# Liaoyongjian1/HC-MVS

Measured on AMD Instinct MI355X. Metric: PatchMatch Mpix/s (1080p, 8 views, 7x7, 8 iter), higher is better.
Workload: dtype f32; 1 GPU; batch of 32 independent units per GPU, each 1 ref x 8 src views, 1920x1080, 7x7 taps (adapthalfwin 6), 8 sweeps, it_external 0, full EstimateDepthMap (median + init score + sweeps + end pass); batch=32, exchange=none

## Files before the change

hc-mvs_amd/csrc/hcmvs_api.cpp:

```cpp
#include "../../include/hcmvs_hip.h"
#include "pm_common.h"
#include "fuse_common.h"
#include "pf_chain.h"
#include "filter_plan.h"
#include "tri_init.h"
#include "cloud_kernels.h"
#include "vis_kernels.h"
#include "dev_buf.h"

#include <cmath>
#include <cstdarg>
#include <cstdio>
#include <cstring>
#include <map>
#include <string>
#include <algorithm>
#include <chrono>
#include <vector>

using namespace hcmvs;

namespace {

constexpr int kMaxBatch = HCMVS_MAX_BATCH;

struct View {
	View() = default;
	explicit View(Reclaimer* r) : grayMem(r), bgrMem(r), gra(r), keep(r), quads(r), depthMem(r), normalMem(r), confMem(r), dNeighbors(r) {}
	int w = 0, h = 0;
	float* gray = nullptr;
	uint8_t* bgr = nullptr;
	DevBuf grayMem, bgrMem;
	DevBuf gra;
	DevBuf keep;
	DevBuf quads;
	double K[9], R[9], C[3];
	float *mDepth = nullptr, *mNormal = nullptr, *mConf = nullptr;
	DevBuf depthMem, normalMem, confMem;
	float dMin = 0.f, dMax = 0.f;
	DevBuf dNeighbors;
	std::vector<uint32_t> neighbors;
	const float *sDepth = nullptr, *sNormal = nullptr, *sConf = nullptr;
	bool rescaled = false;
};

}


struct hcmvs_ctx final : Reclaimer {
	int device = 0;
	hipStream_t ownStream = nullptr;
	hipStream_t stream = nullptr;
	std::string err;
	std::map<uint32_t, View> views;
	struct Slot {
		explicit Slot(Reclaimer* r) : dn(r), conf(r), tmpDepth(r), progress(r), srcSlab(r) {}
		DevBuf dn, conf, tmpDepth;
		DevBuf progress;
		DevBuf srcSlab;
	};
	std::vector<Slot> slots;
	DevBuf tmpU8{this};
	DevBuf maskStage{this};
	DevBuf sDepth{this}, sNormal{this}, sConf{this};
	DevBuf dViews{this};
	std::vector<DevView> hViews;
	DevBuf dItems{this};
	std::vector<EstConst> hItems;
	DevBuf dSpread{this};
	std::vector<SpreadView> hSpread;
	int viewspread = 0;
	bool haveSpreadStats = false;
	DevBuf sync{this};
	int sweepPerLaunch = 0;
	DevBuf evals{this};
	hipEvent_t ev[4] = {nullptr, nullptr, nullptr, nullptr};
	int lastSweeps = 0, lastSweepLaunches = 0;
	bool haveStats = false;
	int sweepLag = 1;
	int sweepSegment = -1;
	int fuseOrder = 0;
	int xcdAffinity = 1;
	DevBuf dMaps{this};
	DevBuf counters{this};
	DevBuf fuseScratch{this};
	DevBuf filterStage{this}, filterTab{this}, filterCnt{this};
	DevBuf passScratch{this};
	DevBuf pfState;
	bool errPending = false;
	int nCU = 0;
	hipEvent_t upEv[2] = {nullptr, nullptr};
	char* pinned = nullptr; size_t capPinned = 0;
	int wavesPerRow = 0;

	bool reclaim() override {
		if (!pfState.capacity()) return false;
		(void)hipStreamSynchronize(stream);
		pfState.reset();
		return true;
	}
};

static int fail(hcmvs_ctx* c, int code, const char* fmt, ...) {
	if (c) {
		char buf[512];
		va_list ap;
		va_start(ap, fmt);
		vsnprintf(buf, sizeof buf, fmt, ap);
		va_end(ap);
		c->err = buf;
	}
	return code;
}
#define HIPCHK(c, call)                                                                             \
	do {                                                                                            \
		hipError_t e_ = (call);                                                                     \
		if (e_ != hipSuccess) return fail(c, HCMVS_ERR_HIP, "%s: %s", #call, hipGetErrorString(e_)); \
	} while (0)

static void mat3_mul(const double* a, const double* b, double* c) {
	for (int i = 0; i < 3; ++i)
		for (int j = 0; j < 3; ++j) {
			double s = 0;
			for (int k = 0; k < 3; ++k) s += a[i * 3 + k] * b[k * 3 + j];
			c[i * 3 + j] = s;
		}
}
static void mat3_mul_bt(const double* a, const double* b, double* c) {
	for (int i = 0; i < 3; ++i)
		for (int j = 0; j < 3; ++j) {
			double s = 0;
			for (int k = 0; k < 3; ++k) s += a[i * 3 + k] * b[j * 3 + k];
			c[i * 3 + j] = s;
		}
}
static void mat3_inv(const double* m, double* r) {
	const double d = m[0] * (m[4] * m[8] - m[5] * m[7]) - m[1] * (m[3] * m[8] - m[5] * m[6]) +
	                 m[2] * (m[3] * m[7] - m[4] * m[6]);
	const double id = 1.0 / d;
	r[0] = (m[4] * m[8] - m[5] * m[7]) * id;
	r[1] = (m[2] * m[7] - m[1] * m[8]) * id;
	r[2] = (m[1] * m[5] - m[2] * m[4]) * id;
	r[3] = (m[5] * m[6] - m[3] * m[8]) * id;
	r[4] = (m[0] * m[8] - m[2] * m[6]) * id;
	r[5] = (m[2] * m[3] - m[0] * m[5]) * id;
	r[6] = (m[3] * m[7] - m[4] * m[6]) * id;
	r[7] = (m[1] * m[6] - m[0] * m[7]) * id;
	r[8] = (m[0] * m[4] - m[1] * m[3]) * id;
}
static inline float fd2r(float d) { return d * (3.14159274101257324f / 180.f); }

#ifdef HCMVS_STAMPS
namespace hcmvs { void debug_read_stamps(unsigned long long* out, int reset); }
#endif
namespace hcmvs {
void launch_resize_gray(const float* src, int sw, int sh, float* dst, int dw, int dh, float scaleParam, hipStream_t s);
void launch_ignore_mask(const uint16_t* labels, int lw, int lh, const int32_t* ignore, int nIgnore, uint8_t* keep, int W, int H, hipStream_t s);
}

extern "C" {

void hcmvs_default_params(hcmvs_params* p) {
	if (!p) return;
	memset(p, 0, sizeof *p);
	p->adapthalfwin = 5;
	p->n_estimation_iters = 1;
	p->it_external = 0;
	p->n_external_iters = 1;
	p->propagate_halfwin = 1;
	p->propagate_step = 4;
	p->n_random_iters = 6;
	p->ncc_threshold_keep = 0.55f;
	p->random_depth_ratio = 0.003f;
	p->random_angle1_deg = 16.f;
	p->random_angle2_deg = 10.f;
	p->random_smooth_depth = 0.02f;
	p->random_smooth_normal_deg = 13.f;
	p->random_smooth_bonus = 0.93f;
	p->photometric_flow = 0.f;
	p->seed = 1234;
	p->median_blur = 1;
}

int hcmvs_create(int device, hcmvs_ctx** out) {
	if (!out) return HCMVS_ERR_INVALID;
	*out = nullptr;
	int n = 0;
	if (hipGetDeviceCount(&n) != hipSuccess || n <= 0 || device < 0 || device >= n) return HCMVS_ERR_NO_DEVICE;
	if (hipSetDevice(device) != hipSuccess) return HCMVS_ERR_NO_DEVICE;
	hipDeviceProp_t prop;
	if (hipGetDeviceProperties(&prop, device) != hipSuccess) return HCMVS_ERR_NO_DEVICE;
	if (strncmp(prop.gcnArchName, "gfx950", 6) != 0) return HCMVS_ERR_NO_DEVICE;
	hcmvs_ctx* c = new hcmvs_ctx();
	c->device = device;
	c->nCU = prop.multiProcessorCount;
	if (hipStreamCreateWithFlags(&c->ownStream, hipStreamNonBlocking) != hipSuccess) { hcmvs_destroy(c); return HCMVS_ERR_NO_DEVICE; }
	c->stream = c->ownStream;
	for (auto& e : c->ev)
		if (hipEventCreate(&e) != hipSuccess) { hcmvs_destroy(c); return HCMVS_ERR_NO_DEVICE; }
	c->hViews.resize((size_t)kMaxBatch * kMaxViews); c->hItems.resize(kMaxBatch); c->hSpread.resize((size_t)kMaxBatch * kMaxViews);
	if (c->dViews.reserve(sizeof(DevView) * kMaxViews * kMaxBatch, c->stream) != hipSuccess || c->evals.reserve(64, c->stream) != hipSuccess ||
	    c->dSpread.reserve(sizeof(SpreadView) * kMaxViews * kMaxBatch, c->stream) != hipSuccess ||
	    c->dItems.reserve(sizeof(EstConst) * kMaxBatch, c->stream) != hipSuccess || c->sync.reserve(64 + sizeof(int32_t) * 2 * kMaxBatch, c->stream) != hipSuccess) {
		hcmvs_destroy(c);
		return HCMVS_ERR_NO_DEVICE;
	}
	const char* lag = getenv("HCMVS_SWEEP_LAG");
	if (lag && atoi(lag) >= 1) c->sweepLag = atoi(lag);
	const char* aff = getenv("HCMVS_XCD_AFFINITY");
	if (aff) c->xcdAffinity = atoi(aff) != 0;
	const char* spl = getenv("HCMVS_SWEEP_LAUNCHES");
	if (spl && strcmp(spl, "per-sweep") == 0) c->sweepPerLaunch = 1;
	if (spl && strcmp(spl, "one") == 0) c->sweepPerLaunch = 2;
	const char* sgl = getenv("HCMVS_SWEEP_SEGMENT");
	if (sgl && atoi(sgl) >= 0) c->sweepSegment = atoi(sgl);
	const char* wpr = getenv("HCMVS_WAVES_PER_ROW");
	if (wpr && (atoi(wpr) == 1 || atoi(wpr) == 2 || atoi(wpr) == 3 || atoi(wpr) == 4)) c->wavesPerRow = atoi(wpr);
	*out = c;
	return HCMVS_OK;
}

void hcmvs_destroy(hcmvs_ctx* c) {
	if (!c) return;
	(void)hipSetDevice(c->device);
	(void)hipStreamSynchronize(c->stream);
	for (auto& e : c->ev) if (e) (void)hipEventDestroy(e);
	if (c->pinned) (void)hipHostFree(c->pinned);
	for (auto& e : c->upEv) if (e) (void)hipEventDestroy(e);
	if (c->ownStream) (void)hipStreamDestroy(c->ownStream);
	delete c;
}

const char* hcmvs_last_error(const hcmvs_ctx* c) { return c ? c->err.c_str() : "null context"; }

static int check_sweep_error(hcmvs_ctx* c) {
	if (!c->errPending) return HCMVS_OK;
	int32_t flags[2] = {0, 0};
	HIPCHK(c, hipMemcpy(flags, c->sync.get(), sizeof flags, hipMemcpyDeviceToHost));
	c->errPending = false;
	if (flags[1] != 0) return fail(c, HCMVS_ERR_TIMEOUT, "sweep worker timed out waiting for its predecessor row; the maps of the last estimate are incomplete");
	return HCMVS_OK;
}

int hcmvs_set_stream(hcmvs_ctx* c, void* stream) {
	if (!c) return HCMVS_ERR_INVALID;
	c->stream = stream ? (hipStream_t)stream : c->ownStream;
	return HCMVS_OK;
}
int hcmvs_synchronize(hcmvs_ctx* c) {
	if (!c) return HCMVS_ERR_INVALID;
	HIPCHK(c, hipSetDevice(c->device));
	HIPCHK(c, hipStreamSynchronize(c->stream));
	return check_sweep_error(c);
}

static int upload_staged(hcmvs_ctx* c, void* dst, const void* src, size_t bytes) {
	{
		hipPointerAttribute_t at;
		if (hipPointerGetAttributes(&at, src) == hipSuccess && at.type == hipMemoryTypeHost) {
			HIPCHK(c, hipMemcpyAsync(dst, src, bytes, hipMemcpyHostToDevice, c->stream));
			HIPCHK(c, hipStreamSynchronize(c->stream));
			return HCMVS_OK;
		}
		(void)hipGetLastError();
	}
	const size_t piece = (size_t)32 << 20;
	if (c->capPinned < 2 * piece) {
		if (c->pinned) (void)hipHostFree(c->pinned);
		c->pinned = nullptr; c->capPinned = 0;
		if (hipHostMalloc((void**)&c->pinned, 2 * piece, hipHostMallocDefault) != hipSuccess) {
			(void)hipGetLastError();
			HIPCHK(c, hipMemcpyAsync(dst, src, bytes, hipMemcpyHostToDevice, c->stream));
			HIPCHK(c, hipStreamSynchronize(c->stream));
			return HCMVS_OK;
		}
		c->capPinned = 2 * piece;
	}
	for (auto& e : c->upEv) if (!e) HIPCHK(c, hipEventCreateWithFlags(&e, hipEventDisableTiming));
	hipEvent_t done[2] = {c->upEv[0], c->upEv[1]};
	bool used[2] = {false, false};
	int k = 0;
	for (size_t off = 0; off < bytes; off += piece, k ^= 1) {
		const size_t n = std::min(piece, bytes - off);
		if (used[k]) HIPCHK(c, hipEventSynchronize(done[k]));
		memcpy(c->pinned + (size_t)k * piece, (const char*)src + off, n);
		HIPCHK(c, hipMemcpyAsync((char*)dst + off, c->pinned + (size_t)k * piece, n, hipMemcpyHostToDevice, c->stream));
		HIPCHK(c, hipEventRecord(done[k], c->stream));
		used[k] = true;
	}
	HIPCHK(c, hipStreamSynchronize(c->stream));
	return HCMVS_OK;
}

static int set_view(hcmvs_ctx* c, uint32_t id, int w, int h, const float* gray, const uint8_t* bgr, const double* K,
                    const double* R, const double* C, bool copy) {
	if (!c) return HCMVS_ERR_INVALID;
	if ((!gray && !bgr) || !K || !R || !C || w < 2 * kHalfWindow + 2 || h < 2 * kHalfWindow + 2 || w > 32768 || h > 32768 || id >= 65536)
		return fail(c, HCMVS_ERR_INVALID, "upload_view: bad arguments (id %u, %dx%d)", id, w, h);
	HIPCHK(c, hipSetDevice(c->device));
	auto it = c->views.find(id);
	if (it != c->views.end()) { HIPCHK(c, hipStreamSynchronize(c->stream)); it->second = View(c); }
	View v(c);
	v.w = w; v.h = h;
	const size_t n = (size_t)w * h;
	if (copy) {
		if (gray) {
			HIPCHK(c, v.grayMem.reserve(n * sizeof(float), c->stream));
			v.gray = v.grayMem.get<float>();
			const int rc = upload_staged(c, v.gray, gray, n * sizeof(float));
			if (rc) return rc;
		}
		if (bgr) {
			HIPCHK(c, v.bgrMem.reserve(n * 3, c->stream));
			v.bgr = v.bgrMem.get<uint8_t>();
			const int rc = upload_staged(c, v.bgr, bgr, n * 3);
			if (rc) return rc;
		}
	} else {
		v.gray = const_cast<float*>(gray);
		v.bgr = const_cast<uint8_t*>(bgr);
	}
	memcpy(v.K, K, sizeof v.K); memcpy(v.R, R, sizeof v.R); memcpy(v.C, C, sizeof v.C);
	c->views[id] = std::move(v);
	return HCMVS_OK;
}

int hcmvs_upload_view(hcmvs_ctx* c, uint32_t id, int32_t w, int32_t h, const float* gray, const uint8_t* bgr,
                      const double K[9], const double R[9], const double C[3]) {
	return set_view(c, id, w, h, gray, bgr, K, R, C, true);
}
int hcmvs_set_view_device(hcmvs_ctx* c, uint32_t id, int32_t w, int32_t h, const float* gray, const uint8_t* bgr,
                          const double K[9], const double R[9], const double C[3]) {
	return set_view(c, id, w, h, gray, bgr, K, R, C, false);
}
int hcmvs_rescale_view(hcmvs_ctx* c, uint32_t src_id, uint32_t dst_id, float scale) {
	if (!c) return HCMVS_ERR_INVALID;
	auto it = c->views.find(src_id);
	if (it == c->views.end() || dst_id >= 65536 || dst_id == src_id) return fail(c, HCMVS_ERR_INVALID, "rescale_view: bad view ids %u -> %u", src_id, dst_id);
	if (!(scale > 0.f) || fabsf(scale - 1.f) < 0.15f) return fail(c, HCMVS_ERR_INVALID, "rescale_view: scale %g is within 15 %% of 1 (DepthMap.h:234: not resampled)", scale);
	const View& src = it->second;
	if (!src.gray) return fail(c, HCMVS_ERR_INVALID, "rescale_view: view %u has no gray image (fuse-only view)", src_id);
	const int nw = (int)lrint((double)src.w * (double)scale), nh = (int)lrint((double)src.h * (double)scale);
	if (nw < 2 * kHalfWindow + 2 || nh < 2 * kHalfWindow + 2 || nw > 32768 || nh > 32768) return fail(c, HCMVS_ERR_INVALID, "rescale_view: %dx%d x %g gives an unusable size", src.w, src.h, scale);
	HIPCHK(c, hipSetDevice(c->device));
	auto old = c->views.find(dst_id);
	if (old != c->views.end()) { HIPCHK(c, hipStreamSynchronize(c->stream)); c->views.erase(old); }
	View v(c);
	v.w = nw; v.h = nh;
	HIPCHK(c, v.grayMem.reserve((size_t)nw * nh * sizeof(float), c->stream));
	v.gray = v.grayMem.get<float>();
	hcmvs::launch_resize_gray(src.gray, src.w, src.h, v.gray, nw, nh, scale, c->stream);
	HIPCHK(c, hipGetLastError());
	const double f = (double)std::max(nw, nh) / (double)std::max(src.w, src.h);
	memcpy(v.K, src.K, sizeof v.K); memcpy(v.R, src.R, sizeof v.R); memcpy(v.C, src.C, sizeof v.C);
	v.K[0] *= f; v.K[4] *= f; v.K[2] *= f; v.K[5] *= f;
	v.rescaled = true;
	c->views[dst_id] = std::move(v);
	return HCMVS_OK;
}
int hcmvs_get_view_info(hcmvs_ctx* c, uint32_t id, int32_t* w, int32_t* h, double K[9]) {
	if (!c) return HCMVS_ERR_INVALID;
	auto it = c->views.find(id);
	if (it == c->views.end()) return fail(c, HCMVS_ERR_INVALID, "get_view_info: unknown view %u", id);
	if (w) *w = it->second.w;
	if (h) *h = it->second.h;
	if (K) memcpy(K, it->second.K, sizeof(double) * 9);
	return HCMVS_OK;
}
int hcmvs_get_view_gray(hcmvs_ctx* c, uint32_t id, float* out) {
	if (!c || !out) return HCMVS_ERR_INVALID;
	auto it = c->views.find(id);
	if (it == c->views.end() || !it->second.gray) return fail(c, HCMVS_ERR_INVALID, "get_view_gray: unknown view %u (or a fuse-only view)", id);
	HIPCHK(c, hipSetDevice(c->device));
	HIPCHK(c, hipMemcpyAsync(out, it->second.gray, (size_t)it->second.w * it->second.h * sizeof(float), hipMemcpyDeviceToHost, c->stream));
	HIPCHK(c, hipStreamSynchronize(c->stream));
	return HCMVS_OK;
}

int hcmvs_release_view(hcmvs_ctx* c, uint32_t id) {
	if (!c) return HCMVS_ERR_INVALID;
	auto it = c->views.find(id);
	if (it == c->views.end()) return fail(c, HCMVS_ERR_INVALID, "release_view: unknown view %u", id);
	HIPCHK(c, hipSetDevice(c->device));
	HIPCHK(c, hipStreamSynchronize(c->stream));
	c->views.erase(it);
	return HCMVS_OK;
}

static int ensure_slot(hcmvs_ctx* c, int i, size_t n, int rows) {
	while ((int)c->slots.size() <= i) c->slots.emplace_back(c);
	hcmvs_ctx::Slot& sl = c->slots[i];
	HIPCHK(c, sl.dn.reserve(n * sizeof(float4), c->stream));
	HIPCHK(c, sl.conf.reserve(n * sizeof(float), c->stream));
	HIPCHK(c, sl.tmpDepth.reserve(n * sizeof(float), c->stream));
	HIPCHK(c, sl.progress.reserve((size_t)rows * kProgressStride * sizeof(int32_t), c->stream));
	return HCMVS_OK;
}

static int ensure_gradient(hcmvs_ctx* c, View& v) {
	if (v.gra.capacity()) return HCMVS_OK;
	const int n = v.w * v.h;
	HIPCHK(c, c->tmpU8.reserve((size_t)n, c->stream));
	HIPCHK(c, v.gra.reserve((size_t)n, c->stream));
	if (v.bgr) launch_bgr_to_u8(v.bgr, c->tmpU8.get<uint8_t>(), n, c->stream);
	else launch_gray_to_u8(v.gray, c->tmpU8.get<uint8_t>(), n, c->stream);
	launch_gradient_map(c->tmpU8.get<uint8_t>(), v.gra.get<uint8_t>(), v.w, v.h, c->stream);
	HIPCHK(c, hipGetLastError());
	return HCMVS_OK;
}

static int ensure_quads(hcmvs_ctx* c, View& v) {
	if (v.quads.capacity()) return HCMVS_OK;
	HIPCHK(c, v.quads.reserve((size_t)v.w * v.h * sizeof(float4), c->stream));
	launch_quads(v.gray, v.quads.get<float4>(), v.w, v.h, c->stream);
	HIPCHK(c, hipGetLastError());
	return HCMVS_OK;
}

int hcmvs_get_gradient_map(hcmvs_ctx* c, uint32_t id, uint8_t* out) {
	if (!c || !out) return HCMVS_ERR_INVALID;
	auto it = c->views.find(id);
	if (it == c->views.end()) return fail(c, HCMVS_ERR_INVALID, "get_gradient_map: unknown view %u", id);
	HIPCHK(c, hipSetDevice(c->device));
	int rc = ensure_gradient(c, it->second);
	if (rc) return rc;
	HIPCHK(c, hipMemcpyAsync(out, it->second.gra.get(), (size_t)it->second.w * it->second.h, hipMemcpyDeviceToHost, c->stream));
	HIPCHK(c, hipStreamSynchronize(c->stream));
	return HCMVS_OK;
}

static int set_ignore_mask(hcmvs_ctx* c, uint32_t id, const uint16_t* labels, int32_t lw, int32_t lh, const int32_t* ignore, int32_t nIgnore,
                           bool device) {
	if (!c) return HCMVS_ERR_INVALID;
	auto it = c->views.find(id);
	if (it == c->views.end()) return fail(c, HCMVS_ERR_INVALID, "set_ignore_mask: unknown view %u", id);
	View& v = it->second;
	HIPCHK(c, hipSetDevice(c->device));
	if (!labels) {
		HIPCHK(c, hipStreamSynchronize(c->stream));
		v.keep.reset();
		return HCMVS_OK;
	}
	if (lw < 1 || lh < 1 || lw > 65536 || lh > 65536 || nIgnore < 0 || (nIgnore > 0 && !ignore))
		return fail(c, HCMVS_ERR_INVALID, "set_ignore_mask: bad arguments (view %u, label image %dx%d, %d labels)", id, lw, lh, nIgnore);
	std::vector<int32_t> lab;
	for (int i = 0; i < nIgnore; ++i)
		if (ignore[i] >= 0 && ignore[i] <= 65535 && std::find(lab.begin(), lab.end(), ignore[i]) == lab.end()) lab.push_back(ignore[i]);
	const size_t imgBytes = (size_t)lw * lh * sizeof(uint16_t);
	Carve cv;
	const size_t oImg = device ? 0 : cv(imgBytes), oLab = cv(sizeof(int32_t) * (lab.size() + 1));
	HIPCHK(c, c->maskStage.reserve(cv.size, c->stream));
	HIPCHK(c, v.keep.reserve((size_t)v.w * v.h, c->stream));
	const uint16_t* dLabels = labels;
	if (!device) {
		const int rc = upload_staged(c, c->maskStage.get() + oImg, labels, imgBytes);
		if (rc) return rc;
		dLabels = (const uint16_t*)(c->maskStage.get() + oImg);
	}
	int32_t* dIgnore = (int32_t*)(c->maskStage.get() + oLab);
	if (!lab.empty()) HIPCHK(c, hipMemcpyAsync(dIgnore, lab.data(), sizeof(int32_t) * lab.size(), hipMemcpyHostToDevice, c->stream));
	launch_ignore_mask(dLabels, lw, lh, dIgnore, (int)lab.size(), v.keep.get<uint8_t>(), v.w, v.h, c->stream);
	HIPCHK(c, hipGetLastError());
	HIPCHK(c, hipStreamSynchronize(c->stream));
	return HCMVS_OK;
}

int hcmvs_set_ignore_mask(hcmvs_ctx* c, uint32_t id, const uint16_t* labels, int32_t lw, int32_t lh, const int32_t* ignore, int32_t n_ignore) {
	return set_ignore_mask(c, id, labels, lw, lh, ignore, n_ignore, false);
}
int hcmvs_set_ignore_mask_device(hcmvs_ctx* c, uint32_t id, const uint16_t* d_labels, int32_t lw, int32_t lh, const int32_t* ignore,
                                 int32_t n_ignore) {
	return set_ignore_mask(c, id, d_labels, lw, lh, ignore, n_ignore, true);
}
int hcmvs_get_ignore_mask(hcmvs_ctx* c, uint32_t id, uint8_t* keep) {
	if (!c || !keep) return HCMVS_ERR_INVALID;
	auto it = c->views.find(id);
	if (it == c->views.end()) return fail(c, HCMVS_ERR_INVALID, "get_ignore_mask: unknown view %u", id);
	const View& v = it->second;
	if (!v.keep.capacity()) { memset(keep, 1, (size_t)v.w * v.h); return HCMVS_OK; }
	HIPCHK(c, hipSetDevice(c->device));
	HIPCHK(c, hipMemcpyAsync(keep, v.keep.get(), (size_t)v.w * v.h, hipMemcpyDeviceToHost, c->stream));
	HIPCHK(c, hipStreamSynchronize(c->stream));
	return HCMVS_OK;
}

static int build_item(hcmvs_ctx* c, int slot, const hcmvs_batch_item& it, const hcmvs_params* p, EstConst& k) {
	if (!it.src_ids || !it.d_depth || !it.d_normal || !it.d_conf) return fail(c, HCMVS_ERR_INVALID, "estimate: null argument");
	const int n_src = it.n_src;
	if (n_src < 1 || n_src > HCMVS_MAX_VIEWS) return fail(c, HCMVS_ERR_INVALID, "estimate: n_src %d not in 1..%d", n_src, HCMVS_MAX_VIEWS);
	if (!(it.d_min >= 0.f) || !(it.d_max > it.d_min)) return fail(c, HCMVS_ERR_INVALID, "estimate: bad depth range [%g,%g)", it.d_min, it.d_max);
	auto rit = c->views.find(it.ref_id);
	if (rit == c->views.end()) return fail(c, HCMVS_ERR_INVALID, "estimate: unknown reference view %u", it.ref_id);
	View& ref = rit->second;
	if (!ref.gray) return fail(c, HCMVS_ERR_INVALID, "estimate: view %u was registered without a gray image (fuse-only view)", it.ref_id);
	int rc = ensure_slot(c, slot, (size_t)ref.w * ref.h, ref.h);
	if (rc) return rc;
	rc = ensure_gradient(c, ref);
	if (rc) return rc;
	memset(&k, 0, sizeof k);
	k.W = ref.w; k.H = ref.h; k.V = n_src;
	k.border = p->adapthalfwin > kHalfWindow ? p->adapthalfwin : kHalfWindow;
	if (ref.w < 2 * k.border + 2 || ref.h < 2 * k.border + 2) return fail(c, HCMVS_ERR_INVALID, "estimate: view %u (%dx%d) has no pixel inside the %d px border", it.ref_id, ref.w, ref.h, k.border);
	k.adapthalfwin = p->adapthalfwin; k.nRandomIters = p->n_random_iters; k.itExternal = p->it_external;
	k.propHalfwin = p->propagate_halfwin; k.propStep = p->propagate_step;
	k.ref = ref.gray; k.gra = ref.gra.get<uint8_t>(); k.views = c->dViews.get<DevView>() + (size_t)slot * kMaxViews;
	double Hr[9];
	mat3_inv(ref.K, Hr);
	for (int i = 0; i < 9; ++i) k.Hr[i] = (float)Hr[i];
	k.ifx = 1.0 / ref.K[0]; k.ify = 1.0 / ref.K[4]; k.cx = ref.K[2]; k.cy = ref.K[5];
	DevView* hv = c->hViews.data() + (size_t)slot * kMaxViews;
	memset(hv, 0, sizeof(DevView) * kMaxViews);
	uintptr_t lo = ~(uintptr_t)0, hi = 0;
	for (int v = 0; v < n_src; ++v) {
		auto sit = c->views.find(it.src_ids[v]);
		if (sit == c->views.end()) return fail(c, HCMVS_ERR_INVALID, "estimate: unknown source view %u", it.src_ids[v]);
		View& s = sit->second;
		if (!s.gray) return fail(c, HCMVS_ERR_INVALID, "estimate: source view %u was registered without a gray image (fuse-only view)", it.src_ids[v]);
		rc = ensure_quads(c, s);
		if (rc) return rc;
		double KR[9], Hl[9], A[9];
		mat3_mul(s.K, s.R, KR);
		mat3_mul_bt(KR, ref.R, Hl);
		const double dC[3] = {ref.C[0] - s.C[0], ref.C[1] - s.C[1], ref.C[2] - s.C[2]};
		for (int i = 0; i < 3; ++i) hv[v].Hm[i] = (float)(KR[i * 3] * dC[0] + KR[i * 3 + 1] * dC[1] + KR[i * 3 + 2] * dC[2]);
		mat3_mul(Hl, Hr, A);
		for (int i = 0; i < 9; ++i) hv[v].A[i] = (float)A[i];
		hv[v].w = s.w; hv[v].h = s.h;
		const uintptr_t b = (uintptr_t)s.quads.get(), e = b + (size_t)s.w * s.h * sizeof(float4);
		if (b < lo) lo = b;
		if (e > hi) hi = e;
	}
	if (hi - lo < 0xFFFF0000ull) {
		k.imgBase = (const char*)lo;
		for (int v = 0; v < n_src; ++v) hv[v].byteOff = (uint32_t)((uintptr_t)c->views.find(it.src_ids[v])->second.quads.get() - lo);
	} else {
		Carve slab;
		for (int v = 0; v < n_src; ++v) { const View& s = c->views.find(it.src_ids[v])->second; hv[v].byteOff = (uint32_t)slab((size_t)s.w * s.h * sizeof(float4)); }
		if (slab.size >= 0xFFFF0000ull) return fail(c, HCMVS_ERR_INVALID, "estimate: the source images of one item exceed 4 GiB");
		DevBuf& srcSlab = c->slots[slot].srcSlab;
		HIPCHK(c, srcSlab.reserve(slab.size, c->stream));
		for (int v = 0; v < n_src; ++v) {
			const View& s = c->views.find(it.src_ids[v])->second;
			HIPCHK(c, hipMemcpyAsync(srcSlab.get() + hv[v].byteOff, s.quads.get(), (size_t)s.w * s.h * sizeof(float4), hipMemcpyDeviceToDevice, c->stream));
		}
		k.imgBase = srcSlab.get();
	}
	k.dMin = it.d_min; k.dMax = it.d_max; k.dMinSqr = sqrtf(it.d_min); k.dMaxSqr = sqrtf(it.d_max);
	k.smoothBonusDepth = 1.f - p->random_smooth_bonus;
	k.smoothBonusNormal = (1.f - p->random_smooth_bonus) * 0.96f;
	k.smoothSigmaDepth = -1.f / (2.f * (p->random_smooth_depth * p->random_smooth_depth));
	{ const float r = fd2r(p->random_smooth_normal_deg); k.smoothSigmaNormal = -1.f / (2.f * (r * r)); }
	k.angle1Range = fd2r(p->random_angle1_deg);
	k.angle2Range = fd2r(p->random_angle2_deg);
	k.thConfSmall = p->ncc_threshold_keep * 0.2f;
	k.thConfBig = p->ncc_threshold_keep * 0.4f;
	k.thConfRand = p->ncc_threshold_keep * 0.9f;
	k.thRobust = p->ncc_threshold_keep * 1.2f;
	k.thKeep = p->ncc_threshold_keep;
	k.depthRatio = p->random_depth_ratio;
	k.pfScale = 1.f - p->photometric_flow;
	k.seed = p->seed + it.seed_offset;
	k.dn = c->slots[slot].dn.get<float4>(); k.conf = c->slots[slot].conf.get<float>(); k.progress = c->slots[slot].progress.get<int32_t>();
	k.hintDepth = nullptr; k.hintNormal = nullptr; k.hintIter = -1;
	if (it.d_hint_depth && it.d_hint_normal && p->it_external == p->n_external_iters - 1) {
		k.hintDepth = it.d_hint_depth; k.hintNormal = it.d_hint_normal; k.hintIter = p->n_estimation_iters - 1;
	}
	k.keep = ref.keep.capacity() ? ref.keep.get<uint8_t>() : nullptr;
	k.spread = nullptr;
	SpreadView* hs = c->hSpread.data() + (size_t)slot * kMaxViews;
	memset(hs, 0, sizeof(SpreadView) * kMaxViews);
	if (c->viewspread && p->it_external >= 1) {
		bool any = false;
		for (int v = 0; v < n_src; ++v) {
			const View& s = c->views.find(it.src_ids[v])->second;
			if (!s.sDepth || s.rescaled) continue;
			any = true;
			hs[v].depth = s.sDepth; hs[v].normal = s.sNormal; hs[v].conf = s.sConf;
			hs[v].w = s.w; hs[v].h = s.h;
			hs[v].cx = s.K[2]; hs[v].cy = s.K[5]; hs[v].ifx = 1.0 / s.K[0]; hs[v].ify = 1.0 / s.K[4];
			double T[9];
			mat3_mul_bt(ref.R, s.R, T);
			const double dC[3] = {s.C[0] - ref.C[0], s.C[1] - ref.C[1], s.C[2] - ref.C[2]};
			hs[v].Tz[0] = T[6]; hs[v].Tz[1] = T[7]; hs[v].Tz[2] = T[8];
			hs[v].tz = ref.R[6] * dC[0] + ref.R[7] * dC[1] + ref.R[8] * dC[2];
		}
		if (any) k.spread = c->dSpread.get<SpreadView>() + (size_t)slot * kMaxViews;
	}
	return HCMVS_OK;
}

static inline bool overlaps(const void* a, size_t na, const void* b, size_t nb) {
	const uintptr_t a0 = (uintptr_t)a, b0 = (uintptr_t)b;
	return a0 < b0 + nb && b0 < a0 + na;
}

static int check_spread_overlap(hcmvs_ctx* c, const hcmvs_batch_item* items, int n_items) {
	for (int i = 0; i < n_items; ++i) {
		const size_t n = (size_t)c->hItems[i].W * c->hItems[i].H;
		for (int k = 0; k < n_items; ++k)
			for (int v = 0; v < items[k].n_src; ++v) {
				const SpreadView& sv = c->hSpread[(size_t)k * kMaxViews + v];
				if (!c->hItems[k].spread || !sv.depth) continue;
				const size_t m = (size_t)sv.w * sv.h;
				const void* io[3] = {items[i].d_depth, items[i].d_normal, items[i].d_conf};
				const size_t ion[3] = {n * 4, n * 12, n * 4};
				const void* sp[3] = {sv.depth, sv.normal, sv.conf};
				const size_t spn[3] = {m * 4, m * 12, m * 4};
				for (int a = 0; a < 3; ++a)
					for (int b = 0; b < 3; ++b)
						if (overlaps(io[a], ion[a], sp[b], spn[b]))
							return fail(c, HCMVS_ERR_INVALID, "estimate: the in/out maps of item %d (view %u) overlap the spread maps of source view %u of item %d: "
							            "a launch must not read what it writes (register a copy, or estimate the two images in separate calls)", i, items[i].ref_id, items[k].src_ids[v], k);
			}
	}
	return HCMVS_OK;
}

int hcmvs_estimate_batch_device(hcmvs_ctx* c, const hcmvs_batch_item* items, int32_t n_items, const hcmvs_params* p) {
	if (!c) return HCMVS_ERR_INVALID;
	if (!items || !p) return fail(c, HCMVS_ERR_INVALID, "estimate: null argument");
	if (n_items < 1 || n_items > kMaxBatch) return fail(c, HCMVS_ERR_INVALID, "estimate: batch size %d not in 1..%d", n_items, kMaxBatch);
	if (p->adapthalfwin < 1 || p->adapthalfwin > kMaxHalfWindow) return fail(c, HCMVS_ERR_INVALID, "estimate: adapthalfwin %d not in 1..%d", p->adapthalfwin, kMaxHalfWindow);
	if (p->n_estimation_iters < 0 || p->n_random_iters < 0 || p->n_random_iters > 20)
		return fail(c, HCMVS_ERR_INVALID, "estimate: bad iteration counts");
	HIPCHK(c, hipSetDevice(c->device));
	int maxRows = 0;
	bool spread = false;
	hcmvs::SweepBatch batch;
	batch.big = p->adapthalfwin > kHalfWindow; batch.nSweeps = p->n_estimation_iters; batch.nCU = c->nCU;
	batch.sweepPerLaunch = c->sweepPerLaunch; batch.sweepSegment = c->sweepSegment; batch.wavesPerRow = c->wavesPerRow;
	for (int i = 0; i < n_items; ++i) {
		if (items[i].n_src < 1 || items[i].n_src > kMaxViews || hcmvs::segments_for(items[i].n_src) != hcmvs::segments_for(items[0].n_src))
			return fail(c, HCMVS_ERR_INVALID, "estimate: the items of a batch must use source-view counts of one class (1-8 or 9-16)");
		int rc = build_item(c, i, items[i], p, c->hItems[i]);
		if (rc) return rc;
		const EstConst& k = c->hItems[i];
		const int rows = k.H - 2 * k.border;
		if (rows > maxRows) maxRows = rows;
		spread = spread || k.spread;
		batch.items.push_back({rows, k.W - 2 * k.border, k.V, k.hintDepth && k.hintIter == batch.nSweeps - 1, k.keep != nullptr, k.spread != nullptr});
	}
	if (spread) { int rc = check_spread_overlap(c, items, n_items); if (rc) return rc; }
	hipStream_t s = c->stream;
	if (spread) HIPCHK(c, hipMemcpyAsync(c->dSpread.get(), c->hSpread.data(), sizeof(SpreadView) * kMaxViews * n_items, hipMemcpyHostToDevice, s));
	c->haveSpreadStats = spread;
	HIPCHK(c, hipMemcpyAsync(c->dViews.get(), c->hViews.data(), sizeof(DevView) * kMaxViews * n_items, hipMemcpyHostToDevice, s));
	HIPCHK(c, hipMemcpyAsync(c->dItems.get(), c->hItems.data(), sizeof(EstConst) * n_items, hipMemcpyHostToDevice, s));
	HIPCHK(c, hipMemsetAsync(c->evals.get(), 0, 64, s));
	HIPCHK(c, hipMemsetAsync(c->sync.get(), 0, 64 + sizeof(int32_t) * 2 * kMaxBatch, s));

	HIPCHK(c, hipEventRecord(c->ev[0], s));
	for (int i = 0; i < n_items; ++i) {
		const EstConst& k = c->hItems[i];
		const float* depthIn = items[i].d_depth;
		if (k.keep) launch_apply_mask(k.keep, items[i].d_depth, items[i].d_normal, k.W * k.H, s);
		if (p->median_blur) {
			launch_median3(items[i].d_depth, c->slots[i].tmpDepth.get<float>(), k.W, k.H, s);
			depthIn = c->slots[i].tmpDepth.get<float>();
		}
		launch_score_pass(k, depthIn, items[i].d_normal, c->evals.get<unsigned long long>(), s);
	}
	HIPCHK(c, hipEventRecord(c->ev[1], s));
	int32_t* sync = c->sync.get<int32_t>();
	const SweepArgs sa{c->dItems.get<EstConst>(), n_items, maxRows, {sync + 16, sync + 16 + kMaxBatch, sync + 1, c->evals.get<unsigned long long>()}, c->sweepLag, c->xcdAffinity};
	const std::vector<hcmvs::SweepLaunch> plan = hcmvs::plan_sweeps(batch);
	for (const hcmvs::SweepLaunch& l : plan) {
		HIPCHK(c, hipMemsetAsync(sync + 16, 0, sizeof(int32_t) * 2 * kMaxBatch, s));
		for (int i = 0; i < n_items; ++i)
			HIPCHK(c, hipMemsetAsync(c->slots[i].progress.get(), 0, (size_t)batch.items[i].rows * kProgressStride * sizeof(int32_t), s));
		if (!launch_sweep(sa, l, s))
			return fail(c, HCMVS_ERR_INVALID, "estimate: no sweep kernel for %d waves per row, big %d two %d pack %d hint %d mask %d spread %d",
			            l.v.nw, l.v.big, l.v.two, l.v.pack, l.v.hint, l.v.mask, l.v.spread);
	}
	c->lastSweepLaunches = (int)plan.size();
	HIPCHK(c, hipEventRecord(c->ev[2], s));
	for (int i = 0; i < n_items; ++i)
		launch_end_pass(c->hItems[i], p->it_external == p->n_external_iters - 1 ? 1 : 0, items[i].d_depth, items[i].d_normal, items[i].d_conf, s);
	HIPCHK(c, hipEventRecord(c->ev[3], s));
	HIPCHK(c, hipGetLastError());
	c->lastSweeps = p->n_estimation_iters;
	c->haveStats = true;
	c->errPending = true;
	return HCMVS_OK;
}

int hcmvs_estimate_device(hcmvs_ctx* c, uint32_t ref_id, const uint32_t* src_ids, int32_t n_src, const hcmvs_params* p,
                          float d_min, float d_max, float* d_depth, float* d_normal, float* d_conf) {
	hcmvs_batch_item it;
	memset(&it, 0, sizeof it);
	it.ref_id = ref_id; it.src_ids = src_ids; it.n_src = n_src; it.d_min = d_min; it.d_max = d_max;
	it.d_depth = d_depth; it.d_normal = d_normal; it.d_conf = d_conf; it.seed_offset = 0;
	return hcmvs_estimate_batch_device(c, &it, 1, p);
}

int hcmvs_get_stats(hcmvs_ctx* c, hcmvs_stats* out) {
	if (!c || !out) return HCMVS_ERR_INVALID;
	memset(out, 0, sizeof *out);
	if (!c->haveStats) return fail(c, HCMVS_ERR_INVALID, "get_stats: no estimate has run");
	HIPCHK(c, hipSetDevice(c->device));
	HIPCHK(c, hipStreamSynchronize(c->stream));
	unsigned long long ev[4] = {0, 0, 0, 0};
	HIPCHK(c, hipMemcpy(ev, c->evals.get(), 32, hipMemcpyDeviceToHost));
	out->evals = ev[0];
	out->evals_issued = ev[1];
	out->tap_evals = ev[2];
	HIPCHK(c, hipEventElapsedTime(&out->ms_score, c->ev[0], c->ev[1]));
	HIPCHK(c, hipEventElapsedTime(&out->ms_sweeps, c->ev[1], c->ev[2]));
	HIPCHK(c, hipEventElapsedTime(&out->ms_end, c->ev[2], c->ev[3]));
	HIPCHK(c, hipEventElapsedTime(&out->ms_total, c->ev[0], c->ev[3]));
	out->n_sweeps = c->lastSweeps;
	out->n_sweep_launches = c->lastSweepLaunches;
	out->ms_sweep_avg = c->lastSweeps > 0 ? out->ms_sweeps / (float)c->lastSweeps : 0.f;
	c->errPending = true;
	return check_sweep_error(c);
}


int hcmvs_set_viewspread(hcmvs_ctx* c, int32_t on) {
	if (!c) return HCMVS_ERR_INVALID;
	c->viewspread = on != 0;
	return HCMVS_OK;
}
int hcmvs_set_spread_maps_device(hcmvs_ctx* c, uint32_t id, const float* d_depth, const float* d_normal, const float* d_conf) {
	if (!c) return HCMVS_ERR_INVALID;
	auto it = c->views.find(id);
	if (it == c->views.end()) return fail(c, HCMVS_ERR_INVALID, "set_spread_maps: unknown view %u", id);
	View& v = it->second;
	if (!d_depth && !d_normal && !d_conf) { v.sDepth = v.sNormal = v.sConf = nullptr; return HCMVS_OK; }
	if (!d_depth || !d_normal || !d_conf) return fail(c, HCMVS_ERR_INVALID, "set_spread_maps: view %u: depth, normal and conf are all needed (or all NULL)", id);
	if (v.rescaled) return fail(c, HCMVS_ERR_INVALID, "set_spread_maps: view %u was made by hcmvs_rescale_view: a resampled view has no maps of its size and never spreads", id);
	v.sDepth = d_depth; v.sNormal = d_normal; v.sConf = d_conf;
	return HCMVS_OK;
}
int hcmvs_get_spread_stats(hcmvs_ctx* c, hcmvs_spread_stats* out) {
	if (!c || !out) return HCMVS_ERR_INVALID;
	memset(out, 0, sizeof *out);
	if (!c->haveStats) return fail(c, HCMVS_ERR_INVALID, "get_spread_stats: no estimate has run");
	if (!c->haveSpreadStats) return HCMVS_OK;
	HIPCHK(c, hipSetDevice(c->device));
	HIPCHK(c, hipStreamSynchronize(c->stream));
	unsigned long long ev[8];
	HIPCHK(c, hipMemcpy(ev, c->evals.get(), 64, hipMemcpyDeviceToHost));
	out->slots_scored = ev[4]; out->slots_accepted = ev[5]; out->slots_dropped = ev[6]; out->candidates_outside = ev[7];
	return HCMVS_OK;
}

int hcmvs_estimate(hcmvs_ctx* c, uint32_t ref_id, const uint32_t* src_ids, int32_t n_src, const hcmvs_params* p, float d_min,
                   float d_max, float* depth, float* normal, float* conf) {
	if (!c) return HCMVS_ERR_INVALID;
	if (!depth || !normal || !conf) return fail(c, HCMVS_ERR_INVALID, "estimate: null map buffer");
	auto rit = c->views.find(ref_id);
	if (rit == c->views.end()) return fail(c, HCMVS_ERR_INVALID, "estimate: unknown reference view %u", ref_id);
	HIPCHK(c, hipSetDevice(c->device));
	const size_t n = (size_t)rit->second.w * rit->second.h;
	hipStream_t s = c->stream;
	HIPCHK(c, c->sDepth.reserve(n * 4, s));
	HIPCHK(c, c->sNormal.reserve(n * 12, s));
	HIPCHK(c, c->sConf.reserve(n * 4, s));
	float *sDepth = c->sDepth.get<float>(), *sNormal = c->sNormal.get<float>(), *sConf = c->sConf.get<float>();
	HIPCHK(c, hipMemcpyAsync(sDepth, depth, n * 4, hipMemcpyHostToDevice, s));
	HIPCHK(c, hipMemcpyAsync(sNormal, normal, n * 12, hipMemcpyHostToDevice, s));
	HIPCHK(c, hipMemcpyAsync(sConf, conf, n * 4, hipMemcpyHostToDevice, s));
	int rc = hcmvs_estimate_device(c, ref_id, src_ids, n_src, p, d_min, d_max, sDepth, sNormal, sConf);
	if (rc) return rc;
	HIPCHK(c, hipMemcpyAsync(depth, sDepth, n * 4, hipMemcpyDeviceToHost, s));
	HIPCHK(c, hipMemcpyAsync(normal, sNormal, n * 12, hipMemcpyDeviceToHost, s));
	HIPCHK(c, hipMemcpyAsync(conf, sConf, n * 4, hipMemcpyDeviceToHost, s));
	HIPCHK(c, hipStreamSynchronize(s));
	hcmvs_stats st;
	return hcmvs_get_stats(c, &st);
}

int hcmvs_splat_points(int32_t W, int32_t H, const double K[9], const double R[9], const double C[3], const float* pts, int32_t n, float* depth,
                       float* normal, float* d_min, float* d_max) {
	if (!K || !R || !C || !pts || !depth || !normal || !d_min || !d_max || n < 1 || W < 1 || H < 1) return HCMVS_ERR_INVALID;
	memset(depth, 0, sizeof(float) * (size_t)W * H);
	float dmin = 3.402823466e+38f, dmax = 0.f;
	for (int i = 0; i < n; ++i) {
		const double X[3] = {pts[3 * i] - C[0], pts[3 * i + 1] - C[1], pts[3 * i + 2] - C[2]};
		double cam[3];
		for (int r = 0; r < 3; ++r) cam[r] = R[r * 3] * X[0] + R[r * 3 + 1] * X[1] + R[r * 3 + 2] * X[2];
		const int x = (int)std::floor(K[2] + K[0] * (cam[0] / cam[2]) + .5);
		const int y = (int)std::floor(K[5] + K[4] * (cam[1] / cam[2]) + .5);
		const float d = (float)cam[2];
		const int sx = x - 2 > 0 ? x - 2 : 0, sy = y - 2 > 0 ? y - 2 : 0;
		const int ex = x + 2 < W - 1 ? x + 2 : W - 1, ey = y + 2 < H - 1 ? y + 2 : H - 1;
		for (int yy = sy; yy <= ey; ++yy)
			for (int xx = sx; xx <= ex; ++xx) {
				depth[(size_t)yy * W + xx] = d;
				float* nn = normal + 3 * ((size_t)yy * W + xx);
				nn[0] = nn[1] = nn[2] = 0.f;
			}
		if (dmin > d) dmin = d;
		if (dmax < d) dmax = d;
	}
	*d_min = dmin * 0.9f;
	*d_max = dmax * 1.1f;
	return HCMVS_OK;
}
int hcmvs_splat_init(hcmvs_ctx* c, uint32_t id, const float* pts, int32_t n, float* depth, float* normal, float* d_min,
                     float* d_max) {
	if (!c) return HCMVS_ERR_INVALID;
	if (!pts || !depth || !normal || !d_min || !d_max || n < 1) return fail(c, HCMVS_ERR_INVALID, "splat_init: bad arguments");
	auto it = c->views.find(id);
	if (it == c->views.end()) return fail(c, HCMVS_ERR_INVALID, "splat_init: unknown view %u", id);
	const View& v = it->second;
	return hcmvs_splat_points(v.w, v.h, v.K, v.R, v.C, pts, n, depth, normal, d_min, d_max);
}

int hcmvs_triangulate_points(int32_t W, int32_t H, const double K[9], const double R[9], const double C[3], const float* pts,
                             int32_t n, float avg_depth, int32_t add_corners, float* depth, float* normal, float* d_min, float* d_max) {
	if (!K || !R || !C || !pts || !depth || !normal || !d_min || !d_max || n < 1 || W < 1 || H < 1) return HCMVS_ERR_INVALID;
	float lo = 0.f, hi = 0.f;
	if (!hcmvs::triangulate_init(W, H, K, R, C, pts, n, avg_depth, add_corners != 0, depth, normal, &lo, &hi)) return HCMVS_ERR_INVALID;
	*d_min = lo * 0.9f;
	*d_max = hi * 1.1f;
	return HCMVS_OK;
}
int hcmvs_triangulate_init(hcmvs_ctx* c, uint32_t id, const float* pts, int32_t n, float avg_depth, int32_t add_corners, float* depth,
                           float* normal, float* d_min, float* d_max) {
	if (!c) return HCMVS_ERR_INVALID;
	if (!pts || !depth || !normal || !d_min || !d_max || n < 1) return fail(c, HCMVS_ERR_INVALID, "triangulate_init: bad arguments");
	auto it = c->views.find(id);
	if (it == c->views.end()) return fail(c, HCMVS_ERR_INVALID, "triangulate_init: unknown view %u", id);
	const View& v = it->second;
	if (hcmvs_triangulate_points(v.w, v.h, v.K, v.R, v.C, pts, n, avg_depth, add_corners, depth, normal, d_min, d_max) != HCMVS_OK)
		return fail(c, HCMVS_ERR_INVALID, "triangulate_init: no sparse point in front of view %u", id);
	return HCMVS_OK;
}

int hcmvs_resize_area_up(const float* src, int32_t sw, int32_t sh, int32_t ch, float* dst, int32_t dw, int32_t dh) {
	if (!src || !dst || sw < 1 || sh < 1 || ch < 1 || dw < sw || dh < sh) return HCMVS_ERR_INVALID;
	struct Tab { std::vector<int> ofs; std::vector<float> w; };
	auto table = [](int ssize, int dsize, bool columns) {
		Tab t; t.ofs.resize((size_t)dsize); t.w.resize((size_t)dsize);
		const double scale = (double)ssize / dsize, inv = (double)dsize / ssize;
		for (int d = 0; d < dsize; ++d) {
			int s = (int)std::floor(d * scale);
			float f = (float)((d + 1) - (s + 1) * inv);
			f = f <= 0 ? 0.f : f - std::floor(f);
			if (columns && s >= ssize - 1) { f = 0.f; s = ssize - 1; }
			t.ofs[(size_t)d] = s; t.w[(size_t)d] = f;
		}
		return t;
	};
	const Tab tx = table(sw, dw, true), ty = table(sh, dh, false);
	std::vector<float> row0((size_t)dw * ch), row1((size_t)dw * ch);
	auto hresize = [&](int sy, std::vector<float>& out) {
		const float* S = src + (size_t)sy * sw * ch;
		for (int x = 0; x < dw; ++x) {
			const int sx = tx.ofs[(size_t)x];
			const float a1 = tx.w[(size_t)x], a0 = 1.f - a1;
			for (int c = 0; c < ch; ++c)
				out[(size_t)x * ch + c] = sx + 1 >= sw ? S[(size_t)sx * ch + c] : S[(size_t)sx * ch + c] * a0 + S[(size_t)(sx + 1) * ch + c] * a1;
		}
	};
	int have0 = -1, have1 = -1;
	for (int y = 0; y < dh; ++y) {
		const int r0 = std::min(std::max(ty.ofs[(size_t)y], 0), sh - 1), r1 = std::min(std::max(ty.ofs[(size_t)y] + 1, 0), sh - 1);
		if (have0 != r0) { if (have1 == r0) { row0.swap(row1); std::swap(have0, have1); } else { hresize(r0, row0); have0 = r0; } }
		if (have1 != r1) { hresize(r1, row1); have1 = r1; }
		const float b1 = ty.w[(size_t)y], b0 = 1.f - b1;
		float* D = dst + (size_t)y * dw * ch;
		for (size_t k = 0; k < (size_t)dw * ch; ++k) D[k] = row0[k] * b0 + row1[k] * b1;
	}
	return HCMVS_OK;
}


static int set_maps(hcmvs_ctx* c, uint32_t id, const float* depth, const float* normal, const float* conf, float dmin, float dmax, bool copy) {
	if (!c) return HCMVS_ERR_INVALID;
	auto it = c->views.find(id);
	if (it == c->views.end()) return fail(c, HCMVS_ERR_INVALID, "set_depthmap: unknown view %u", id);
	if (!depth || !conf) return fail(c, HCMVS_ERR_INVALID, "set_depthmap: null map");
	View& v = it->second;
	HIPCHK(c, hipSetDevice(c->device));
	HIPCHK(c, hipStreamSynchronize(c->stream));
	v.mDepth = v.mNormal = v.mConf = nullptr;
	v.depthMem.reset(); v.normalMem.reset(); v.confMem.reset();
	const size_t n = (size_t)v.w * v.h;
	if (copy) {
		HIPCHK(c, v.depthMem.reserve(n * 4, c->stream));
		HIPCHK(c, v.confMem.reserve(n * 4, c->stream));
		v.mDepth = v.depthMem.get<float>(); v.mConf = v.confMem.get<float>();
		int rc = upload_staged(c, v.mDepth, depth, n * 4);
		if (!rc) rc = upload_staged(c, v.mConf, conf, n * 4);
		if (rc) return rc;
		if (normal) {
			HIPCHK(c, v.normalMem.reserve(n * 12, c->stream));
			v.mNormal = v.normalMem.get<float>();
			rc = upload_staged(c, v.mNormal, normal, n * 12);
			if (rc) return rc;
		}
	} else {
		v.mDepth = const_cast<float*>(depth); v.mNormal = const_cast<float*>(normal); v.mConf = const_cast<float*>(conf);
	}
	v.dMin = dmin; v.dMax = dmax;
	return HCMVS_OK;
}
int hcmvs_set_depthmap(hcmvs_ctx* c, uint32_t id, const float* depth, const float* normal, const float* conf, float d_min, float d_max) {
	return set_maps(c, id, depth, normal, conf, d_min, d_max, true);
}
int hcmvs_set_depthmap_device(hcmvs_ctx* c, uint32_t id, float* d_depth, const float* d_normal, const float* d_conf, float d_min, float d_max) {
	return set_maps(c, id, d_depth, d_normal, d_conf, d_min, d_max, false);
}
int hcmvs_get_depthmap(hcmvs_ctx* c, uint32_t id, float* depth, float* normal, float* conf) {
	if (!c) return HCMVS_ERR_INVALID;
	auto it = c->views.find(id);
	if (it == c->views.end() || !it->second.mDepth) return fail(c, HCMVS_ERR_INVALID, "get_depthmap: view %u has no maps", id);
	const View& v = it->second;
	const size_t n = (size_t)v.w * v.h;
	HIPCHK(c, hipSetDevice(c->device));
	HIPCHK(c, hipStreamSynchronize(c->stream));
	if (depth) HIPCHK(c, hipMemcpy(depth, v.mDepth, n * 4, hipMemcpyDeviceToHost));
	if (normal && v.mNormal) HIPCHK(c, hipMemcpy(normal, v.mNormal, n * 12, hipMemcpyDeviceToHost));
	if (conf) HIPCHK(c, hipMemcpy(conf, v.mConf, n * 4, hipMemcpyDeviceToHost));
	return HCMVS_OK;
}
int hcmvs_set_neighbors(hcmvs_ctx* c, uint32_t id, const uint32_t* ids, int32_t n) {
	if (!c) return HCMVS_ERR_INVALID;
	auto it = c->views.find(id);
	if (it == c->views.end() || n < 0 || n > 64 || (n > 0 && !ids)) return fail(c, HCMVS_ERR_INVALID, "set_neighbors: bad arguments for view %u", id);
	View& v = it->second;
	HIPCHK(c, hipSetDevice(c->device));
	HIPCHK(c, hipStreamSynchronize(c->stream));
	v.dNeighbors.reset();
	v.neighbors.assign(ids, ids + n);
	if (n > 0) {
		HIPCHK(c, v.dNeighbors.reserve((size_t)n * 4, c->stream));
		HIPCHK(c, hipMemcpy(v.dNeighbors.get(), ids, (size_t)n * 4, hipMemcpyHostToDevice));
	}
	return HCMVS_OK;
}

static void fill_devmap(uint32_t id, const View& v, DevMap& m) {
	memset(&m, 0, sizeof m);
	m.id = id; m.w = v.w; m.h = v.h; m.nNeighbors = (int)v.neighbors.size();
	memcpy(m.K, v.K, sizeof m.K); memcpy(m.R, v.R, sizeof m.R); memcpy(m.C, v.C, sizeof m.C);
	double t[3];
	for (int i = 0; i < 3; ++i) t[i] = -(v.R[i * 3] * v.C[0] + v.R[i * 3 + 1] * v.C[1] + v.R[i * 3 + 2] * v.C[2]);
	for (int i = 0; i < 3; ++i) {
		for (int j = 0; j < 3; ++j) m.P[i * 4 + j] = v.K[i * 3] * v.R[j] + v.K[i * 3 + 1] * v.R[3 + j] + v.K[i * 3 + 2] * v.R[6 + j];
		m.P[i * 4 + 3] = v.K[i * 3] * t[0] + v.K[i * 3 + 1] * t[1] + v.K[i * 3 + 2] * t[2];
	}
	m.depth = v.mDepth; m.normal = v.mNormal; m.conf = v.mConf; m.bgr = v.bgr;
	m.neighbors = v.dNeighbors.get<uint32_t>(); m.dMin = v.dMin; m.dMax = v.dMax;
}
static int build_map_table(hcmvs_ctx* c, std::vector<DevMap>& host) {
	uint32_t maxId = 0;
	for (auto& kv : c->views) if (kv.first > maxId) maxId = kv.first;
	host.assign((size_t)maxId + 1, DevMap());
	for (auto& m : host) memset(&m, 0, sizeof m);
	for (auto& kv : c->views) fill_devmap(kv.first, kv.second, host[kv.first]);
	HIPCHK(c, c->dMaps.reserve(host.size() * sizeof(DevMap), c->stream));
	HIPCHK(c, hipMemcpy(c->dMaps.get(), host.data(), host.size() * sizeof(DevMap), hipMemcpyHostToDevice));
	HIPCHK(c, c->counters.reserve(8 * sizeof(unsigned long long), c->stream));
	return HCMVS_OK;
}

int hcmvs_filter(hcmvs_ctx* c, uint32_t ref_id, const uint32_t* nbr, int32_t N, int32_t adjust, int32_t n_min_views,
                 int32_t n_min_views_adjust, float depth_diff_threshold, float* out_depth, float* out_conf, uint64_t* n_processed,
                 uint64_t* n_discarded) {
	if (!c) return HCMVS_ERR_INVALID;
	if (!nbr || !out_depth || !out_conf || N < 1 || N > 64) return fail(c, HCMVS_ERR_INVALID, "filter: bad arguments");
	if (N < n_min_views || N < n_min_views_adjust) return fail(c, HCMVS_ERR_INVALID, "filter: depth map %u can not be filtered (%d neighbours)", ref_id, N);
	HIPCHK(c, hipSetDevice(c->device));
	HIPCHK(c, hipStreamSynchronize(c->stream));
	std::vector<DevMap> host;
	int rc = build_map_table(c, host);
	if (rc) return rc;
	if (ref_id >= host.size() || !host[ref_id].depth) return fail(c, HCMVS_ERR_INVALID, "filter: view %u has no maps", ref_id);
	std::vector<DevMap> nbs((size_t)N);
	for (int n = 0; n < N; ++n) {
		if (nbr[n] >= host.size() || !host[nbr[n]].depth) return fail(c, HCMVS_ERR_INVALID, "filter: neighbour %u has no maps", nbr[n]);
		nbs[n] = host[nbr[n]];
	}
	const DevMap& ref = host[ref_id];
	const size_t area = (size_t)ref.w * ref.h;
	const size_t offNb = area * N * 8, offD = offNb + ((sizeof(DevMap) * N + 255) & ~(size_t)255), offC = offD + area * 4;
	HIPCHK(c, c->fuseScratch.reserve(offC + area * 4, c->stream));
// ... 572 lines not shown
```

hc-mvs_amd/csrc/pm_common.h:

```cpp
#ifndef HCMVS_PM_COMMON_H
#define HCMVS_PM_COMMON_H

#include <hip/hip_runtime.h>
#include <stdint.h>
#include <utility>
#include "sweep_plan.h"

namespace hcmvs {

constexpr int kHalfWindow = 7;
constexpr int kMaxHalfWindow = 10;
constexpr int kBigTaps = (kMaxHalfWindow + 1) * (kMaxHalfWindow + 1);
constexpr int kBigSlots = 128;
constexpr int kMaxViews = 16;
constexpr int kMaxSlots = 32;
constexpr int kProgressStride = 16;

struct DevView {
	uint32_t byteOff;
	int32_t w, h;
	float A[9];
	float Hm[3];
};

struct SpreadView {
	const float* depth;
	const float* normal;
	const float* conf;
	int32_t w, h;
	double cx, cy, ifx, ify;
	double Tz[3], tz;
};

struct EstConst {
	int32_t W, H, V;
	int32_t border;
	int32_t adapthalfwin, nRandomIters, itExternal, propHalfwin, propStep;
	const float* ref;
	const uint8_t* gra;
	const DevView* views;
	const char* imgBase;
	float Hr[9];
	double cx, cy, ifx, ify;
	float dMin, dMax, dMinSqr, dMaxSqr;
	float smoothBonusDepth, smoothBonusNormal, smoothSigmaDepth, smoothSigmaNormal;
	float angle1Range, angle2Range;
	float thConfSmall, thConfBig, thConfRand, thRobust, thKeep;
	float depthRatio, pfScale;
	uint32_t seed;
	float4* dn;
	float* conf;
	int32_t* progress;
	const float* hintDepth;
	const float* hintNormal;
	int32_t hintIter;
	const uint8_t* keep;
	const SpreadView* spread;
};

struct SweepSync {
	int32_t* ticket;
	int32_t* rowsDone;
	int32_t* error;
	unsigned long long* evals;
};

struct SweepArgs {
	const EstConst* dItems;
	int nItems, maxRows;
	SweepSync sync;
	int lag, affinity;
};

void launch_gray_to_u8(const float* gray, uint8_t* out, int n, hipStream_t s);
void launch_bgr_to_u8(const uint8_t* bgr, uint8_t* out, int n, hipStream_t s);
void launch_gradient_map(const uint8_t* g8, uint8_t* gra, int W, int H, hipStream_t s);
void launch_median3(const float* in, float* out, int W, int H, hipStream_t s);
void launch_apply_mask(const uint8_t* keep, float* depth, float* normal, int n, hipStream_t s);
void launch_quads(const float* gray, float4* out, int W, int H, hipStream_t s);
void launch_score_pass(const EstConst& c, const float* depthIn, const float* normalIn, unsigned long long* evals,
                       hipStream_t s);
bool launch_sweep(const SweepArgs& a, const SweepLaunch& l, hipStream_t s);
void launch_end_pass(const EstConst& c, int finalPass, float* depth, float* normal, float* conf, hipStream_t s);

}
#endif
```

hc-mvs_amd/csrc/pm_kernels.hip:

```cpp
#include "pm_common.h"
#include "pm_math.h"

#include <float.h>
#include <type_traits>

namespace hcmvs {

#define HC_SQ(x) ((x) * (x))

#ifdef HCMVS_STAMPS
__device__ unsigned long long g_stamps[32];
#define STAMP_DECL unsigned long long st_last = __builtin_amdgcn_s_memtime(), st_acc[16] = {0, 0, 0, 0, 0, 0, 0, 0, 0, 0, 0, 0, 0, 0, 0, 0}; unsigned st_cnt[16] = {0, 0, 0, 0, 0, 0, 0, 0, 0, 0, 0, 0, 0, 0, 0, 0};
#define STAMP(i) { const unsigned long long t_ = __builtin_amdgcn_s_memtime(); st_acc[i] += t_ - st_last; st_last = t_; }
#define STAMP_ARGS , unsigned long long& st_last, unsigned long long (&st_acc)[16], unsigned (&st_cnt)[16]
#define STAMP_PASS , st_last, st_acc, st_cnt
#define STAMP_FLUSH if ((threadIdx.x & 63) == 0 && (threadIdx.x >> 6) == 0) { for (int i_ = 0; i_ < 16; ++i_) atomicAdd(&g_stamps[i_], st_acc[i_]); for (int i_ = 0; i_ < 16; ++i_) atomicAdd(&g_stamps[16 + i_], (unsigned long long)st_cnt[i_]); }
#define SUBMARK(name)
#define BLOCK(name, i) ++st_cnt[i];
#define BLOCKN(name, i, n) st_cnt[i] += (unsigned)(n);
#elif defined(HCMVS_MARK)
#define STAMP_DECL
#define STAMP(i) asm volatile("; HCMARK " #i);
#define SUBMARK(name) asm volatile("; HCMARK " #name);
#define BLOCK(name, i) asm volatile("; HCMARK " #name);
// ... 1150 lines not shown
			const int t = lane & 3;
			const int cnx = ix + (t == 2 ? -1 : (t == 3 ? 1 : 0)), cny = iy + (t == 0 ? -1 : (t == 1 ? 1 : 0));
			const bool cand = rim && lane < 4;
			const bool inMap = cnx < sw && cny < shh;
			const bool ld = cand && inMap;
			const size_t nidx = ld ? (size_t)cny * (size_t)sw + (size_t)cnx : 0;
			const float sd = sdep[nidx], scf = scnf[nidx];
			const float sn0 = snrm[3 * nidx], sn1 = snrm[3 * nidx + 1], sn2 = snrm[3 * nidx + 2];
			const bool slotV = ld && sd > 0.f;
			const double z = sd;
			const double Xc0 = ((double)cnx - sv[j].cx) * z * sv[j].ifx, Xc1 = ((double)cny - sv[j].cy) * z * sv[j].ify;
			const float zt = (float)(((sv[j].Tz[0] * Xc0 + sv[j].Tz[1] * Xc1) + sv[j].Tz[2] * z) + sv[j].tz);
			const bool open = slotV && !(scf >= c.thKeep);
			const bool hv = open && zt > 0.f;
			float k0 = sn0, k1 = sn1, k2 = sn2;
			if (hv) correct_normal(G, k0, k1, k2);
			closeMask = __ballot(slotV);
			eligMask = __ballot(hv);
			if (wv == 0) {
				spc.outside += (unsigned)__builtin_popcountll(__ballot(cand && !inMap));
				spc.dropped += (unsigned)__builtin_popcountll(__ballot(open && !hv));
			}
			if (lane < kMaxSlots) {
				cl[0][lane] = (float)Xc0; cl[1][lane] = (float)Xc1; cl[2][lane] = sd;
				cl[3][lane] = sn0; cl[4][lane] = sn1; cl[5][lane] = sn2;
				cl[6][lane] = k0; cl[7][lane] = k1; cl[8][lane] = k2;
			}
			if (eligMask == 0ull) continue;
			const int src = (lane >> 3) < 4 ? (lane >> 3) : 0;
			const float gd = __shfl(zt, src, 64), g0 = __shfl(k0, src, 64), g1 = __shfl(k1, src, 64), g2 = __shfl(k2, src, 64);
			const float gpd = -gd * dot3(g0, g1, g2, G.v0, G.v1, 1.f);
			const float F = smooth_pass(c, cl, closeMask, eligMask, lane, gd, g0, g1, g2, g0, g1, g2, gpd, src);
			float s1 = __builtin_huge_valf(), s2 = __builtin_huge_valf();
			score_chunk<S, BIG, PACK>(c, L, P, st, G.v0, G.v1, F, zt, k0, k1, k2, eligMask, 0, __builtin_ctzll(eligMask), s1, s2, issued);
			if constexpr (TWO) {
				unsigned again = 0;
				score_chunk<S, BIG, PACK>(c, L1, P, st, G.v0, G.v1, F, zt, k0, k1, k2, eligMask, 0, __builtin_ctzll(eligMask), s1, s2, again);
			}
			const float all = two_best(c, s1, s2);
			for (unsigned long long mk = eligMask; mk; mk &= mk - 1ull) {
				const int i = __builtin_ctzll(mk);
				const float nconf = rlf(all, i);
				++evals;
				if (wv == 0) ++spc.scored;
				if (conf > nconf) {
					conf = nconf; depth = rlf(zt, i); n0 = rlf(k0, i); n1 = rlf(k1, i); n2 = rlf(k2, i);
					if (wv == 0) ++spc.accepted;
				}
			}
		}
	}
	if constexpr (HINT) if (c.hintDepth && iter == c.hintIter) {
		const float hdep = as_global(c.hintDepth)[idx];
		if (hdep > 0.f) {
			float h0 = as_global(c.hintNormal)[3 * idx], h1 = as_global(c.hintNormal)[3 * idx + 1], h2 = as_global(c.hintNormal)[3 * idx + 2];
			const float hd = interpolate_pixel(c, G, x, y, hdep, h0, h1, h2);
			correct_normal(G, h0, h1, h2);
			const float hpd = -hd * dot3(h0, h1, h2, G.v0, G.v1, 1.f);
			const float F = smooth_pass(c, st.pk->cl, closeMask, eligMask, lane, hd, h0, h1, h2, h0, h1, h2, hpd, 63);
			float s1 = __builtin_huge_valf(), s2 = __builtin_huge_valf();
			score_chunk<S, BIG, PACK>(c, L, P, st, G.v0, G.v1, F, hd, h0, h1, h2, 1ull, 0, 0, s1, s2, issued);
			if constexpr (TWO) {
				unsigned again = 0;
				score_chunk<S, BIG, PACK>(c, L1, P, st, G.v0, G.v1, F, hd, h0, h1, h2, 1ull, 0, 0, s1, s2, again);
			}
			const float nconf = rlf(two_best(c, s1, s2), 0);
			++evals;
			if (conf > nconf - 0.1f) { conf = nconf; depth = hd; n0 = h0; n1 = h1; n2 = h2; }
		}
	}
	if (hooked && !pollTaken && pp.r > 0 && pp.poll > pp.known) pp.known = pp.poll;
	if (lane == 0) {
		float* hrec = sh.hist[q & (kHist - 1)];
		hrec[0] = depth; hrec[1] = n0; hrec[2] = n1; hrec[3] = n2; hrec[4] = conf;
		if (wv == NW - 1) {
			store_dn(&c.dn[idx], depth, n0, n1, n2);
			store_f(&c.conf[idx], conf);
		}
	}
	if constexpr (NW == 1) {
		pp.pendingPub = q + 1;
	} else if (wv == NW - 1) {
		asm volatile("s_waitcnt vmcnt(0)" ::: "memory");
		if (lane == 0) __hip_atomic_store(pp.myWord, pp.base + q + 1, __ATOMIC_RELAXED, HC_SCOPE);
	}
	STAMP(15)

}


#ifndef HCMVS_OCC
#define HCMVS_OCC 3
#endif
template <int S, int NW, bool BIG, bool TWO = false, bool PACK = false, bool HINT = false, bool MASK = false, bool SPREAD = false>
__global__ __launch_bounds__(64 * NW) __attribute__((amdgpu_waves_per_eu(!BIG ? HCMVS_OCC : 1, !BIG ? HCMVS_OCC : 2))) void sweep_kernel(const EstConst* __restrict__ items, int nItems, int maxRows, SweepSync sy,
                                                        int iter0, int nSweeps, int lag, int affinity, int segLen) {
	__shared__ RowShared<NW> sh;
	__shared__ WavePark<S> park[NW];
	__shared__ float bigTab[BIG ? NW : 1][4][BIG ? kBigSlots : 1];
	const int wv = __builtin_amdgcn_readfirstlane((int)(threadIdx.x >> 6));
	unsigned evals = 0, issued = 0;
	unsigned long long taps = 0;
	SpreadCount spc = {0u, 0u, 0u, 0u};
	int par = 0, rot = (int)blockIdx.x;
	STAMP_DECL
	RowPipe<S> pp;
	pp.err = as_global(sy.error);
	for (;;) {
		if (NW > 1) __syncthreads();
		if (threadIdx.x == 0) {
			int item = -1, row = 0;
			const int G = nItems < 8 ? nItems : 8;
			const int home = affinity ? (int)(__builtin_amdgcn_s_getreg(6164) & 7u) % G : 0;
			const int nHome = affinity ? (nItems - home + G - 1) / G : nItems;
			float behind = 2.f;
			if (segLen > 0 && affinity)
				for (int k = 0; k < nItems; ++k) {
					const int nrows_ = items[k].H - 2 * items[k].border;
					const int per_ = nrows_ * ((items[k].W - 2 * items[k].border + segLen - 1) / segLen);
					const int t_ = __hip_atomic_load(as_global(sy.ticket) + k, __ATOMIC_RELAXED, HC_SCOPE);
					if (t_ < per_ * nSweeps) { const float f = (float)t_ / (float)per_; behind = f < behind ? f : behind; }
				}
			for (int pass = 0; pass < 2 && item < 0; ++pass)
				for (int k = 0; k < nItems && item < 0; ++k) {
					int cand;
					if (!affinity) cand = (rot + k) % nItems;
					else if (k < nHome) cand = home + ((rot + k) % nHome) * G;
					else {
						cand = k - nHome;
						cand += cand / (G - 1) + (cand % (G - 1) >= home ? 1 : 0);
					}
					const int nrows_ = items[cand].H - 2 * items[cand].border;
					const int per_ = nrows_ * (segLen > 0 ? (items[cand].W - 2 * items[cand].border + segLen - 1) / segLen : 1);
					HC_GLOBAL int32_t* tk = as_global(sy.ticket) + cand;
					const int t_ = __hip_atomic_load(tk, __ATOMIC_RELAXED, HC_SCOPE);
					if (t_ >= per_ * nSweeps) continue;
					if (pass == 0 && segLen > 0 && affinity && (float)t_ / (float)per_ > behind + 1.f / 64.f) continue;
					if (pass == 0 && t_ > 0 && t_ % per_ == 0 &&
					    __hip_atomic_load(as_global(sy.rowsDone) + cand, __ATOMIC_RELAXED, HC_SCOPE) < (t_ / per_) * nrows_) continue;
					const int r_ = atomicAdd(sy.ticket + cand, 1);
					if (r_ < per_ * nSweeps) { item = cand; row = r_; }
				}
			++rot;
			sh.row = row; sh.item = item;
		}
		__syncthreads();
		const int itemIdx = __builtin_amdgcn_readfirstlane(sh.item);
		if (itemIdx < 0) break;
		const int ticket = __builtin_amdgcn_readfirstlane(sh.row);
		const EstConst& c = items[itemIdx];
		const int bd = c.border;
		const int nrows = c.H - 2 * bd, ncols = c.W - 2 * bd;
		const int nseg = segLen > 0 ? (ncols + segLen - 1) / segLen : 1;
		const int perSweep = nrows * nseg;
		const int sweep = ticket / perSweep;
		int r = ticket - sweep * perSweep, seg = 0;
		if (nseg > 1) {
			const int tt = r;
			auto before = [&](int k) {
				int n = 0;
				for (int g = 0; g < nseg; ++g) { const int v = k - g * segLen; n += v < 0 ? 0 : (v > nrows ? nrows : v); }
				return n;
			};
			int lo = 0, hi = nrows + (nseg - 1) * segLen;
			while (hi - lo > 1) { const int mid = (lo + hi) >> 1; if (before(mid) <= tt) lo = mid; else hi = mid; }
			const int j = tt - before(lo);
			const int over = lo - nrows + 1;
			const int g0 = over > 0 ? (over + segLen - 1) / segLen : 0;
			seg = g0 + j;
			r = lo - seg * segLen;
		}
		const int q0 = seg * segLen, q1 = nseg > 1 && q0 + segLen < ncols ? q0 + segLen : ncols;
		const int iter = iter0 + sweep;
		const bool rev = (iter & 1) != 0;
		pp.rev = rev; pp.base = sweep << 16;
		LaneCtx<S> L;
		lane_init<S>(c, L);
		LdsStore<S> st;
		st.pk = &park[wv]; st.lane = L.lane; st.view = L.view;
		st.bw = (float (*)[kBigSlots])(BIG ? &bigTab[BIG ? wv : 0][0][0] : nullptr);
		st.put_view(as_global(c.views) + (L.vact ? L.view : 0), L.seg);
		LaneCtx<S> L1 = L;
		if constexpr (TWO) {
			lane_init<S>(c, L1, 64 / S);
			LdsStore<S> s1 = st;
			s1.view = L1.view;
			s1.put_view(as_global(c.views) + (L1.vact ? L1.view : 0), L1.seg);
		}
		const int y = rev ? c.H - 1 - bd - r : bd + r;
		pp.r = r; pp.y = y;
		pp.upWord = as_global(c.progress) + (size_t)(r > 0 ? r - 1 : 0) * kProgressStride;
		pp.myWord = as_global(c.progress) + (size_t)r * kProgressStride;
		pp.known = r > 0 ? 0 : 0x7fffffff;
		pp.poll = 0; pp.pendingPub = 0; pp.fail = false;
		STAMP(10)
		if (q0 > 0) {
			pp.fail = wait_progress(pp.myWord, pp.base + q0, pp.err, pp.base + q0 - 4) < 0;
		}
		STAMP(14)
		if (r > 0 && !pp.fail) {
			const int need = q0 + lag < q1 ? q0 + lag : q1;
			pp.known = wait_progress(pp.upWord, pp.base + need, pp.err, pp.base + q0);
			pp.fail = pp.known < 0;
			pp.known -= pp.base;
		} else if (sweep > 0 && q0 == 0) {
			pp.fail = wait_progress(as_global(sy.rowsDone) + itemIdx, sweep * nrows, pp.err, sweep * nrows - 2) < 0;
		}
		if (!pp.fail && (threadIdx.x == 0) && ncols > 0 && q0 == 0) __hip_atomic_store(pp.myWord, pp.base, __ATOMIC_RELAXED, HC_SCOPE);
		if (q0 > 0 && !pp.fail) {
			const int lane = (int)(threadIdx.x & 63);
			const int col = q0 - 1 - lane;
			if (lane < kHist && col >= 0) {
				const int hx = rev ? c.W - 1 - bd - col : bd + col;
				const float4 hdn = load_dn(&c.dn[y * c.W + hx]);
				const float hcf = load_f(&c.conf[y * c.W + hx]);
				float* hrec = sh.hist[col & (kHist - 1)];
				hrec[0] = hdn.x; hrec[1] = hdn.y; hrec[2] = hdn.z; hrec[3] = hdn.w; hrec[4] = hcf;
			}
			if (NW > 1) __syncthreads();
		}

		const int xs = rev ? c.W - 1 - bd - q0 : bd + q0;
		const int dx = rev ? -1 : 1;
		pp.tx1 = uniform_byte(c.gra, y * c.W + xs);
		{
			PixIn<S> first;
			first.tx = (float)pp.tx1;
			load_patch_inputs<S>(c, L, xs, y, first);
			pp.nI = first.I[0]; pp.nC = first.center;
			pp.tx2 = q0 + 1 < q1 ? uniform_byte(c.gra, y * c.W + xs + dx) : (uint8_t)0;
		}
		STAMP(9)
		for (int q = q0; q < q1 && !pp.fail; ++q) {
			const int x = rev ? c.W - 1 - bd - q : bd + q;
			STAMP(13)
			PixIn<S> in;
			in.tx = (float)pp.tx1;
			prefetch_static<S>(c, L, x, y, q, rev, pp.known >= q + 1, in);
			in.I[0] = pp.nI; in.center = pp.nC;
			if (q + 1 < q1) {
				PixIn<S> nxt;
				nxt.tx = (float)pp.tx2;
				load_patch_inputs<S>(c, L, x + dx, y, nxt);
				pp.nI = nxt.I[0]; pp.nC = nxt.center;
			}
			pp.tx1 = pp.tx2;
			if (q + 2 < q1) pp.tx2 = uniform_byte(c.gra, y * c.W + x + 2 * dx);
			uint8_t km = 1;
			if constexpr (MASK) km = uniform_byte(c.keep ? c.keep : c.gra, y * c.W + x);
			STAMP(12)
			Patch<S> P;
			fill_patch<S, BIG>(c, L, x, y, in, P, st);
			STAMP(1)
			if (pp.known < q + 1) {
				pp.known = wait_progress(pp.upWord, pp.base + q + 1, pp.err);
				if (pp.known < 0) {
					pp.fail = true;
					asm volatile("s_waitcnt vmcnt(0)" : "+v"(pp.nI), "+v"(pp.nC) :: "memory");
					break;
				}
				pp.known -= pp.base;
				prefetch_up<S>(c, in);
			}
			asm volatile("s_waitcnt vmcnt(0)" : "+v"(pp.nI), "+v"(pp.nC) :: "memory");
			STAMP(0)
			if (MASK && c.keep && km == 0) {
				if (L.lane == 0) {
					float* hrec = sh.hist[q & (kHist - 1)];
					hrec[0] = in.cur.x; hrec[1] = in.cur.y; hrec[2] = in.cur.z; hrec[3] = in.cur.w; hrec[4] = in.curConf;
					if (wv == NW - 1) __hip_atomic_store(pp.myWord, pp.base + q + 1, __ATOMIC_RELAXED, HC_SCOPE);
				}
				pp.pendingPub = 0;
				continue;
			}
			const unsigned e0 = evals;
			process_pixel<S, NW, BIG, TWO, PACK, HINT, SPREAD>(c, L, L1, sh, par, wv, x, y, q, iter, in, P, st, pp, evals, issued, spc STAMP_PASS);
			taps += (unsigned long long)(evals - e0) * (unsigned)((P.a + 1) * (P.a + 1));
			STAMP(5)
		}
		if (pp.fail) break;
		if (pp.pendingPub > 0) {
			asm volatile("s_waitcnt vmcnt(0)" ::: "memory");
			if ((threadIdx.x & 63) == 0) __hip_atomic_store(pp.myWord, pp.base + pp.pendingPub, __ATOMIC_RELAXED, HC_SCOPE);
			pp.pendingPub = 0;
		}
		if (NW > 1) __syncthreads();
		if (threadIdx.x == 0 && q1 == c.W - 2 * bd) __hip_atomic_fetch_add(as_global(sy.rowsDone) + itemIdx, 1, __ATOMIC_RELAXED, HC_SCOPE);
	}
	STAMP(10)
	STAMP_FLUSH
	if ((threadIdx.x & 63) == 0) {
		if (wv == 0 && evals) { atomicAdd(sy.evals, (unsigned long long)evals); atomicAdd(sy.evals + 2, taps); }
		if (issued) atomicAdd(sy.evals + 1, (unsigned long long)issued);
		if constexpr (SPREAD) if (wv == 0) {
			if (spc.scored) atomicAdd(sy.evals + 4, (unsigned long long)spc.scored);
			if (spc.accepted) atomicAdd(sy.evals + 5, (unsigned long long)spc.accepted);
			if (spc.dropped) atomicAdd(sy.evals + 6, (unsigned long long)spc.dropped);
			if (spc.outside) atomicAdd(sy.evals + 7, (unsigned long long)spc.outside);
		}
	}
}


__global__ void import_kernel(EstConst c, const float* depthIn, const float* normalIn) {
	const int n = c.W * c.H;
	for (int i = blockIdx.x * blockDim.x + threadIdx.x; i < n; i += gridDim.x * blockDim.x) {
		const int x = i % c.W, y = i / c.W;
		const bool inb = x >= c.border && y >= c.border && x < c.W - c.border && y < c.H - c.border;
		if (c.keep && !c.keep[i]) {
			c.dn[i] = make_float4(depthIn[i], 0.f, 0.f, 0.f);
			c.conf[i] = 0.f;
		} else if (inb) {
			c.dn[i] = make_float4(depthIn[i], normalIn[3 * i], normalIn[3 * i + 1], normalIn[3 * i + 2]);
			c.conf[i] = 2.f;
		} else {
			c.dn[i] = make_float4(0.f, 0.f, 0.f, 0.f);
			c.conf[i] = 2.f;
		}
	}
}

template <int S, bool BIG, bool TWO = false, bool MASK = false>
__global__ __launch_bounds__(256) void score_kernel(EstConst c, unsigned long long* evalsOut) {
	LaneCtx<S> L;
	lane_init<S>(c, L);
	__shared__ float stage[4][3][8][8];
	__shared__ float bigTab[BIG ? 4 : 1][4][BIG ? kBigSlots : 1];
	RegStore<S> st;
	st.stage = stage[threadIdx.x >> 6]; st.seg = L.seg;
	st.bw = (float (*)[kBigSlots])(BIG ? &bigTab[BIG ? (threadIdx.x >> 6) : 0][0][0] : nullptr);
	st.put_view(as_global(c.views) + (L.vact ? L.view : 0), L.seg);
	LaneCtx<S> L1 = L;
	RegStore<S> st1 = st;
	if constexpr (TWO) {
		lane_init<S>(c, L1, 64 / S);
		st1.put_view(as_global(c.views) + (L1.vact ? L1.view : 0), L1.seg);
	}
	const int nrows = c.H - 2 * c.border, ncols = c.W - 2 * c.border;
	const int total = nrows * ncols;
	const int wavesPerBlock = blockDim.x >> 6;
	const int gw = blockIdx.x * wavesPerBlock + (threadIdx.x >> 6), nw = gridDim.x * wavesPerBlock;
	unsigned evals = 0;
	unsigned long long taps = 0;
	const uint32_t stream0 = (uint32_t)c.itExternal * 64u;
	for (int p = gw; p < total; p += nw) {
		const int x = c.border + p % ncols, y = c.border + p / ncols;
		const int idx = y * c.W + x;
		if constexpr (MASK) if (!uniform_byte(c.keep, idx)) continue;
		const uint32_t rk = rand_key(c.seed, (uint32_t)idx, stream0);
		PixIn<S> in;
		in.tx = (float)c.gra[idx];
		load_patch_inputs<S>(c, L, x, y, in);
		Patch<S> P;
		fill_patch<S, BIG>(c, L, x, y, in, P, st);
		PixelGeom G;
		pixel_geom(c, x, y, G);
		const float4 cur = c.dn[idx];
		float d = cur.x, n0 = cur.y, n1 = cur.z, n2 = cur.w;
		if (!(c.dMin <= d && d < c.dMax)) {
			d = random_depth(c, rand_unit(rk, 0u));
			random_normal(G, rand_unit(rk, 1u), rand_unit(rk, 2u), n0, n1, n2);
		} else if (dot3(n0, n1, n2, G.v0, G.v1, 1.f) >= 0.f) {
			random_normal(G, rand_unit(rk, 1u), rand_unit(rk, 2u), n0, n1, n2);
		}
		float m1 = __builtin_huge_valf(), m2 = __builtin_huge_valf();
		score_pixel<S, BIG>(c, L, P, st, G.v0, G.v1, 1.f, d, n0, n1, n2, m1, m2);
		if constexpr (TWO) {
			st1.copy_patch(st);
			score_pixel<S, BIG>(c, L1, P, st1, G.v0, G.v1, 1.f, d, n0, n1, n2, m1, m2);
		}
		const float s = two_best(c, m1, m2);
		++evals;
		taps += (unsigned)((P.a + 1) * (P.a + 1));
		if (L.lane == 0) {
			c.dn[idx] = make_float4(d, n0, n1, n2);
			c.conf[idx] = s;
		}
	}
	if (L.lane == 0 && evals) {
		atomicAdd(evalsOut, (unsigned long long)evals);
		atomicAdd(evalsOut + 1, (unsigned long long)evals);
		atomicAdd(evalsOut + 2, taps);
	}
}

#ifdef HCMVS_COUNT
template <int S>
__global__ void probe_score_kernel(EstConst c, Patch<S> P, RegStore<S> st, float F, float d, float n0, float n1, float n2, float* out) {
	LaneCtx<S> L;
	lane_init<S>(c, L);
	float m1 = __builtin_huge_valf(), m2 = __builtin_huge_valf();
	score_pixel<S, false>(c, L, P, st, 0.1f, 0.2f, F, d, n0, n1, n2, m1, m2);
	out[threadIdx.x] = two_best(c, m1, m2);
}
template __global__ void probe_score_kernel<8>(EstConst, Patch<8>, RegStore<8>, float, float, float, float, float, float*);
__global__ void probe_smooth_kernel(EstConst c, Close C, float* out) {
	__shared__ float cl[9][kMaxSlots];
	for (int k = 0; k < 9; ++k) cl[k][threadIdx.x & 31] = out[k * 64 + threadIdx.x];
	out[threadIdx.x] = smooth_pass(c, cl, C.closeMask, C.eligMask, threadIdx.x & 63, out[0], out[1], out[2], out[3], out[4], out[5], out[6], out[7], 63);
}
template <int S>
__global__ void probe_patch_kernel(EstConst c, PixIn<S> in, Patch<S>* out, RegStore<S>* so) {
	LaneCtx<S> L;
	lane_init<S>(c, L);
	Patch<S> P;
	__shared__ float stage[3][8][8];
	RegStore<S> st;
	st.stage = stage; st.seg = L.seg;
	fill_patch<S, false>(c, L, 100, 100, in, P, st);
	out[threadIdx.x] = P;
	so[threadIdx.x] = st;
}
template __global__ void probe_patch_kernel<8>(EstConst, PixIn<8>, Patch<8>*, RegStore<8>*);
#endif

__global__ void end_kernel(EstConst c, int finalPass, float* depth, float* normal, float* conf) {
	const int n = c.W * c.H;
	for (int i = blockIdx.x * blockDim.x + threadIdx.x; i < n; i += gridDim.x * blockDim.x) {
		float4 v = c.dn[i];
		float cf = c.conf[i];
		if (finalPass && !(c.keep && !c.keep[i])) {
			if (v.x <= 0.f || cf >= c.thKeep) { v = make_float4(0.f, 0.f, 0.f, 0.f); cf = 0.f; }
			else cf = cf >= 1.f ? 0.f : 1.f - cf;
		}
		depth[i] = v.x;
		normal[3 * i] = v.y; normal[3 * i + 1] = v.z; normal[3 * i + 2] = v.w;
		conf[i] = cf;
	}
}


__global__ void gray_to_u8_kernel(const float* g, uint8_t* out, int n) {
	for (int i = blockIdx.x * blockDim.x + threadIdx.x; i < n; i += gridDim.x * blockDim.x) {
		const int r = (int)rintf(g[i] * 255.f);
		out[i] = (uint8_t)(r < 0 ? 0 : (r > 255 ? 255 : r));
	}
}
__global__ void bgr_to_u8_kernel(const uint8_t* bgr, uint8_t* out, int n) {
	for (int i = blockIdx.x * blockDim.x + threadIdx.x; i < n; i += gridDim.x * blockDim.x)
		out[i] = (uint8_t)((bgr[3 * i] * 1868 + bgr[3 * i + 1] * 9617 + bgr[3 * i + 2] * 4899 + 8192) >> 14);
}
__device__ __forceinline__ int reflect101(int i, int n) {
	if (n == 1) return 0;
	while (i < 0 || i >= n) i = i < 0 ? -i : 2 * n - 2 - i;
	return i;
}
__global__ void gradient_kernel(const uint8_t* g, uint8_t* gra, int W, int H) {
	const int x = blockIdx.x * blockDim.x + threadIdx.x, y = blockIdx.y * blockDim.y + threadIdx.y;
	if (x >= W || y >= H) return;
	const int xm = reflect101(x - 1, W), xp = reflect101(x + 1, W), ym = reflect101(y - 1, H), yp = reflect101(y + 1, H);
	const int a00 = g[ym * W + xm], a01 = g[ym * W + x], a02 = g[ym * W + xp];
	const int a10 = g[y * W + xm], a12 = g[y * W + xp];
	const int a20 = g[yp * W + xm], a21 = g[yp * W + x], a22 = g[yp * W + xp];
	int ax = abs((a02 + 2 * a12 + a22) - (a00 + 2 * a10 + a20));
	int ay = abs((a20 + 2 * a21 + a22) - (a00 + 2 * a01 + a02));
	ax = ax > 255 ? 255 : ax; ay = ay > 255 ? 255 : ay;
	const int s2 = ax + ay;
	int r = s2 >> 1;
	if ((s2 & 1) && (r & 1)) r += 1;
	gra[y * W + x] = (uint8_t)(r > 255 ? 255 : r);
}
__global__ void quad_kernel(const float* g, float4* out, int W, int H) {
	const int x = blockIdx.x * blockDim.x + threadIdx.x, y = blockIdx.y * blockDim.y + threadIdx.y;
	if (x >= W || y >= H) return;
	const int x1 = x + 1 < W ? x + 1 : W - 1, y1 = y + 1 < H ? y + 1 : H - 1;
	const float i00 = g[(size_t)y * W + x], i10 = g[(size_t)y * W + x1], i01 = g[(size_t)y1 * W + x], i11 = g[(size_t)y1 * W + x1];
	out[(size_t)y * W + x] = make_float4(i00, i10 - i00, i01, i11 - i01);
}
__global__ void median3_kernel(const float* in, float* out, int W, int H) {
	const int x = blockIdx.x * blockDim.x + threadIdx.x, y = blockIdx.y * blockDim.y + threadIdx.y;
	if (x >= W || y >= H) return;
	float v[9];
	int n = 0;
#pragma unroll
	for (int dy = -1; dy <= 1; ++dy) {
		int yy = y + dy; yy = yy < 0 ? 0 : (yy >= H ? H - 1 : yy);
#pragma unroll
		for (int dx = -1; dx <= 1; ++dx) {
			int xx = x + dx; xx = xx < 0 ? 0 : (xx >= W ? W - 1 : xx);
			v[n++] = in[yy * W + xx];
		}
	}
#define HC_SORT2(a, b) { const float lo = fminf(v[a], v[b]), hi = fmaxf(v[a], v[b]); v[a] = lo; v[b] = hi; }
	HC_SORT2(1, 2) HC_SORT2(4, 5) HC_SORT2(7, 8) HC_SORT2(0, 1) HC_SORT2(3, 4) HC_SORT2(6, 7) HC_SORT2(1, 2) HC_SORT2(4, 5)
	HC_SORT2(7, 8) HC_SORT2(0, 3) HC_SORT2(5, 8) HC_SORT2(4, 7) HC_SORT2(3, 6) HC_SORT2(1, 4) HC_SORT2(2, 5) HC_SORT2(4, 7)
	HC_SORT2(4, 2) HC_SORT2(6, 4) HC_SORT2(4, 2)
#undef HC_SORT2
	out[y * W + x] = v[4];
}
__global__ void apply_mask_kernel(const uint8_t* keep, float* depth, float* normal, int n) {
	for (int i = blockIdx.x * blockDim.x + threadIdx.x; i < n; i += gridDim.x * blockDim.x)
		if (!keep[i]) { depth[i] = 0.f; normal[3 * i] = 0.f; normal[3 * i + 1] = 0.f; normal[3 * i + 2] = 0.f; }
}


#ifdef HCMVS_STAMPS
void debug_read_stamps(unsigned long long* out, int reset) {
	(void)hipMemcpyFromSymbol(out, HIP_SYMBOL(g_stamps), sizeof(unsigned long long) * 32);
	if (reset) { unsigned long long z[32] = {0}; (void)hipMemcpyToSymbol(HIP_SYMBOL(g_stamps), z, sizeof z); }
}
#endif

void launch_gray_to_u8(const float* gray, uint8_t* out, int n, hipStream_t s) {
	hipLaunchKernelGGL(gray_to_u8_kernel, dim3(2048), dim3(256), 0, s, gray, out, n);
}
void launch_bgr_to_u8(const uint8_t* bgr, uint8_t* out, int n, hipStream_t s) {
	hipLaunchKernelGGL(bgr_to_u8_kernel, dim3(2048), dim3(256), 0, s, bgr, out, n);
}
void launch_gradient_map(const uint8_t* g8, uint8_t* gra, int W, int H, hipStream_t s) {
	hipLaunchKernelGGL(gradient_kernel, dim3((W + 63) / 64, (H + 3) / 4), dim3(64, 4), 0, s, g8, gra, W, H);
}
void launch_quads(const float* gray, float4* out, int W, int H, hipStream_t s) {
	hipLaunchKernelGGL(quad_kernel, dim3((W + 63) / 64, (H + 3) / 4), dim3(64, 4), 0, s, gray, out, W, H);
}
void launch_median3(const float* in, float* out, int W, int H, hipStream_t s) {
	hipLaunchKernelGGL(median3_kernel, dim3((W + 63) / 64, (H + 3) / 4), dim3(64, 4), 0, s, in, out, W, H);
}
void launch_apply_mask(const uint8_t* keep, float* depth, float* normal, int n, hipStream_t s) {
	hipLaunchKernelGGL(apply_mask_kernel, dim3(2048), dim3(256), 0, s, keep, depth, normal, n);
}

template <class K, int N>
struct KernelTable { K at[N]; };
using ScoreKernel = void (*)(EstConst, unsigned long long*);
template <int... I>
static constexpr KernelTable<ScoreKernel, sizeof...(I)> score_table(std::integer_sequence<int, I...>) {
	return {{score_kernel<8, (I & 4) != 0, (I & 2) != 0, (I & 1) != 0>...}};
}
static constexpr auto kScoreKernels = score_table(std::make_integer_sequence<int, 8>{});
void launch_score_pass(const EstConst& c, const float* depthIn, const float* normalIn, unsigned long long* evals,
                       hipStream_t s) {
	hipLaunchKernelGGL(import_kernel, dim3(2048), dim3(256), 0, s, c, depthIn, normalIn);
	hipLaunchKernelGGL(kScoreKernels.at[(c.adapthalfwin > kHalfWindow ? 4 : 0) | (c.V > 8 ? 2 : 0) | (c.keep ? 1 : 0)], dim3(4096), dim3(256), 0, s, c, evals);
}

using SweepKernel = void (*)(const EstConst*, int, int, SweepSync, int, int, int, int, int);
constexpr int sweep_variant_index(SweepVariant v) {
	return (v.nw - 1) << 6 | v.big << 5 | v.two << 4 | v.pack << 3 | v.hint << 2 | v.mask << 1 | (int)v.spread;
}
constexpr SweepVariant sweep_variant_at(int i) {
	return {(i >> 6) + 1, (i & 32) != 0, (i & 16) != 0, (i & 8) != 0, (i & 4) != 0, (i & 2) != 0, (i & 1) != 0};
}
template <int I>
static constexpr SweepKernel sweep_instance() {
	constexpr SweepVariant v = sweep_variant_at(I);
	if constexpr (sweep_variant_exists(v)) return sweep_kernel<8, v.nw, v.big, v.two, v.pack, v.hint, v.mask, v.spread>;
	else return nullptr;
}
template <int... I>
static constexpr KernelTable<SweepKernel, sizeof...(I)> sweep_table(std::integer_sequence<int, I...>) { return {{sweep_instance<I>()...}}; }
static constexpr auto kSweepKernels = sweep_table(std::make_integer_sequence<int, 4 * 64>{});

bool launch_sweep(const SweepArgs& a, const SweepLaunch& l, hipStream_t s) {
	const SweepKernel k = sweep_variant_exists(l.v) ? kSweepKernels.at[sweep_variant_index(l.v)] : nullptr;
	if (!k) return false;
	if (l.grid >= 1) hipLaunchKernelGGL(k, dim3(l.grid), dim3(64 * l.v.nw), 0, s, a.dItems, a.nItems, a.maxRows, a.sync, l.first, l.count, a.lag, a.affinity, l.segLen);
	return true;
}

void launch_end_pass(const EstConst& c, int finalPass, float* depth, float* normal, float* conf, hipStream_t s) {
	hipLaunchKernelGGL(end_kernel, dim3(2048), dim3(256), 0, s, c, finalPass, depth, normal, conf);
}

}
```

Before: 22.86 Mpix/s.

## Batch per-item init, score, median and end passes into single multi-item launches

Replaces the per-item loops of median, import, score, end-pass and progress-clear launches with single batched launches indexed by item through a device-side InitItem table. The score kernel is rewritten to walk tiles of all items across the whole batch, with a grid sized from occupancy and blocks grouped into tile classes. Host tables move to a double-buffered pinned buffer so uploads are asynchronous and do not overwrite data still in use. The aim is to cut launch count and the tail idle time of the small per-item score launches. In exchange the score kernel keeps more state live across items and reloads view contexts when it crosses item boundaries.

```diff
diff --git a/hc-mvs_amd/csrc/hcmvs_api.cpp b/hc-mvs_amd/csrc/hcmvs_api.cpp
--- a/hc-mvs_amd/csrc/hcmvs_api.cpp
+++ b/hc-mvs_amd/csrc/hcmvs_api.cpp
@@ -64,11 +64,19 @@
 	DevBuf maskStage{this};
 	DevBuf sDepth{this}, sNormal{this}, sConf{this};
 	DevBuf dViews{this};
-	std::vector<DevView> hViews;
 	DevBuf dItems{this};
-	std::vector<EstConst> hItems;
+	DevBuf dInit{this};
 	DevBuf dSpread{this};
-	std::vector<SpreadView> hSpread;
+	char* hTables = nullptr;
+	bool tablesPinned = false;
+	int tabSet = 0;
+	hipEvent_t tabEv[2] = {nullptr, nullptr};
+	EstConst* hItems = nullptr;
+	InitItem* hInit = nullptr;
+	DevView* hViews = nullptr;
+	SpreadView* hSpread = nullptr;
+	int scoreTileW = 64, scoreTileH = 32;
+	int scoreBlocksPerCU[8] = {-1, -1, -1, -1, -1, -1, -1, -1};
 	int viewspread = 0;
 	bool haveSpreadStats = false;
 	DevBuf sync{this};
@@ -148,6 +156,14 @@
 	r[7] = (m[1] * m[6] - m[0] * m[7]) * id;
 	r[8] = (m[0] * m[4] - m[1] * m[3]) * id;
 }
+static constexpr size_t kTabItems = 0, kTabInit = kTabItems + sizeof(EstConst) * kMaxBatch, kTabViews = kTabInit + sizeof(InitItem) * kMaxBatch,
+                        kTabSpread = kTabViews + sizeof(DevView) * kMaxViews * kMaxBatch, kTabBytes = kTabSpread + sizeof(SpreadView) * kMaxViews * kMaxBatch;
+static void use_table_set(hcmvs_ctx* c, int k) {
+	char* b = c->hTables + (size_t)k * kTabBytes;
+	c->tabSet = k;
+	c->hItems = (EstConst*)(b + kTabItems); c->hInit = (InitItem*)(b + kTabInit);
+	c->hViews = (DevView*)(b + kTabViews); c->hSpread = (SpreadView*)(b + kTabSpread);
+}
 static inline float fd2r(float d) { return d * (3.14159274101257324f / 180.f); }
 
 #ifdef HCMVS_STAMPS
@@ -198,8 +214,15 @@
 	c->stream = c->ownStream;
 	for (auto& e : c->ev)
 		if (hipEventCreate(&e) != hipSuccess) { hcmvs_destroy(c); return HCMVS_ERR_NO_DEVICE; }
-	c->hViews.resize((size_t)kMaxBatch * kMaxViews); c->hItems.resize(kMaxBatch); c->hSpread.resize((size_t)kMaxBatch * kMaxViews);
-	if (c->dViews.reserve(sizeof(DevView) * kMaxViews * kMaxBatch, c->stream) != hipSuccess || c->evals.reserve(64, c->stream) != hipSuccess ||
+	for (auto& e : c->tabEv)
+		if (hipEventCreateWithFlags(&e, hipEventDisableTiming) != hipSuccess) { hcmvs_destroy(c); return HCMVS_ERR_NO_DEVICE; }
+	static_assert(kTabInit % 16 == 0 && kTabViews % 16 == 0 && kTabSpread % 16 == 0 && kTabBytes % 16 == 0, "the tables of a set are aligned");
+	c->tablesPinned = hipHostMalloc((void**)&c->hTables, 2 * kTabBytes, hipHostMallocDefault) == hipSuccess;
+	if (!c->tablesPinned) { (void)hipGetLastError(); c->hTables = (char*)malloc(2 * kTabBytes); }
+	if (!c->hTables) { hcmvs_destroy(c); return HCMVS_ERR_NO_DEVICE; }
+	memset(c->hTables, 0, 2 * kTabBytes);
+	use_table_set(c, 0);
+	if (c->dInit.reserve(sizeof(InitItem) * kMaxBatch, c->stream) != hipSuccess || c->dViews.reserve(sizeof(DevView) * kMaxViews * kMaxBatch, c->stream) != hipSuccess || c->evals.reserve(64, c->stream) != hipSuccess ||
 	    c->dSpread.reserve(sizeof(SpreadView) * kMaxViews * kMaxBatch, c->stream) != hipSuccess ||
 	    c->dItems.reserve(sizeof(EstConst) * kMaxBatch, c->stream) != hipSuccess || c->sync.reserve(64 + sizeof(int32_t) * 2 * kMaxBatch, c->stream) != hipSuccess) {
 		hcmvs_destroy(c);
@@ -216,6 +239,12 @@
 	if (sgl && atoi(sgl) >= 0) c->sweepSegment = atoi(sgl);
 	const char* wpr = getenv("HCMVS_WAVES_PER_ROW");
 	if (wpr && (atoi(wpr) == 1 || atoi(wpr) == 2 || atoi(wpr) == 3 || atoi(wpr) == 4)) c->wavesPerRow = atoi(wpr);
+	const char* stl = getenv("HCMVS_SCORE_TILE");
+	if (stl) {
+		int tw = 0, th = 0;
+		if (strcmp(stl, "0") == 0) { c->scoreTileW = 0; c->scoreTileH = 0; }
+		else if (sscanf(stl, "%dx%d", &tw, &th) == 2 && tw >= 1 && th >= 1 && tw <= 32768 && th <= 32768) { c->scoreTileW = tw; c->scoreTileH = th; }
+	}
 	*out = c;
 	return HCMVS_OK;
 }
@@ -225,6 +254,8 @@
 	(void)hipSetDevice(c->device);
 	(void)hipStreamSynchronize(c->stream);
 	for (auto& e : c->ev) if (e) (void)hipEventDestroy(e);
+	for (auto& e : c->tabEv) if (e) (void)hipEventDestroy(e);
+	if (c->hTables) { if (c->tablesPinned) (void)hipHostFree(c->hTables); else free(c->hTables); }
 	if (c->pinned) (void)hipHostFree(c->pinned);
 	for (auto& e : c->upEv) if (e) (void)hipEventDestroy(e);
 	if (c->ownStream) (void)hipStreamDestroy(c->ownStream);
@@ -508,7 +539,7 @@
 	mat3_inv(ref.K, Hr);
 	for (int i = 0; i < 9; ++i) k.Hr[i] = (float)Hr[i];
 	k.ifx = 1.0 / ref.K[0]; k.ify = 1.0 / ref.K[4]; k.cx = ref.K[2]; k.cy = ref.K[5];
-	DevView* hv = c->hViews.data() + (size_t)slot * kMaxViews;
+	DevView* hv = c->hViews + (size_t)slot * kMaxViews;
 	memset(hv, 0, sizeof(DevView) * kMaxViews);
 	uintptr_t lo = ~(uintptr_t)0, hi = 0;
 	for (int v = 0; v < n_src; ++v) {
@@ -567,7 +598,7 @@
 	}
 	k.keep = ref.keep.capacity() ? ref.keep.get<uint8_t>() : nullptr;
 	k.spread = nullptr;
-	SpreadView* hs = c->hSpread.data() + (size_t)slot * kMaxViews;
+	SpreadView* hs = c->hSpread + (size_t)slot * kMaxViews;
 	memset(hs, 0, sizeof(SpreadView) * kMaxViews);
 	if (c->viewspread && p->it_external >= 1) {
 		bool any = false;
@@ -593,6 +624,8 @@
 	const uintptr_t a0 = (uintptr_t)a, b0 = (uintptr_t)b;
 	return a0 < b0 + nb && b0 < a0 + na;
 }
+
+static inline bool k_two(int n_src) { return n_src > 8; }
 
 static int check_spread_overlap(hcmvs_ctx* c, const hcmvs_batch_item* items, int n_items) {
 	for (int i = 0; i < n_items; ++i) {
@@ -624,58 +657,80 @@
 	if (p->n_estimation_iters < 0 || p->n_random_iters < 0 || p->n_random_iters > 20)
 		return fail(c, HCMVS_ERR_INVALID, "estimate: bad iteration counts");
 	HIPCHK(c, hipSetDevice(c->device));
-	int maxRows = 0;
-	bool spread = false;
+	int maxRows = 0, maxW = 0, maxH = 0, nTiles = 0;
+	bool spread = false, mask = false;
 	hcmvs::SweepBatch batch;
 	batch.big = p->adapthalfwin > kHalfWindow; batch.nSweeps = p->n_estimation_iters; batch.nCU = c->nCU;
 	batch.sweepPerLaunch = c->sweepPerLaunch; batch.sweepSegment = c->sweepSegment; batch.wavesPerRow = c->wavesPerRow;
+	HIPCHK(c, hipEventSynchronize(c->tabEv[c->tabSet ^ 1]));
+	use_table_set(c, c->tabSet ^ 1);
 	for (int i = 0; i < n_items; ++i) {
 		if (items[i].n_src < 1 || items[i].n_src > kMaxViews || hcmvs::segments_for(items[i].n_src) != hcmvs::segments_for(items[0].n_src))
 			return fail(c, HCMVS_ERR_INVALID, "estimate: the items of a batch must use source-view counts of one class (1-8 or 9-16)");
 		int rc = build_item(c, i, items[i], p, c->hItems[i]);
 		if (rc) return rc;
 		const EstConst& k = c->hItems[i];
-		const int rows = k.H - 2 * k.border;
+		const int rows = k.H - 2 * k.border, cols = k.W - 2 * k.border;
 		if (rows > maxRows) maxRows = rows;
+		if (k.W > maxW) maxW = k.W;
+		if (k.H > maxH) maxH = k.H;
 		spread = spread || k.spread;
-		batch.items.push_back({rows, k.W - 2 * k.border, k.V, k.hintDepth && k.hintIter == batch.nSweeps - 1, k.keep != nullptr, k.spread != nullptr});
+		mask = mask || k.keep;
+		batch.items.push_back({rows, cols, k.V, k.hintDepth && k.hintIter == batch.nSweeps - 1, k.keep != nullptr, k.spread != nullptr});
+		InitItem& t = c->hInit[i];
+		memset(&t, 0, sizeof t);
+		t.depthIn = items[i].d_depth;
+		if (p->median_blur) { t.medianIn = items[i].d_depth; t.medianOut = c->slots[i].tmpDepth.get<float>(); t.depthIn = t.medianOut; }
+		t.normalIn = items[i].d_normal;
+		t.depthOut = items[i].d_depth; t.normalOut = items[i].d_normal; t.confOut = items[i].d_conf;
+		t.tw = c->scoreTileW > 0 ? c->scoreTileW : cols; t.th = c->scoreTileW > 0 ? c->scoreTileH : rows;
+		t.tilesX = (cols + t.tw - 1) / t.tw;
+		t.tile0 = nTiles;
+		nTiles += t.tilesX * ((rows + t.th - 1) / t.th);
 	}
 	if (spread) { int rc = check_spread_overlap(c, items, n_items); if (rc) return rc; }
 	hipStream_t s = c->stream;
-	if (spread) HIPCHK(c, hipMemcpyAsync(c->dSpread.get(), c->hSpread.data(), sizeof(SpreadView) * kMaxViews * n_items, hipMemcpyHostToDevice, s));
+	if (spread) HIPCHK(c, hipMemcpyAsync(c->dSpread.get(), c->hSpread, sizeof(SpreadView) * kMaxViews * n_items, hipMemcpyHostToDevice, s));
 	c->haveSpreadStats = spread;
-	HIPCHK(c, hipMemcpyAsync(c->dViews.get(), c->hViews.data(), sizeof(DevView) * kMaxViews * n_items, hipMemcpyHostToDevice, s));
-	HIPCHK(c, hipMemcpyAsync(c->dItems.get(), c->hItems.data(), sizeof(EstConst) * n_items, hipMemcpyHostToDevice, s));
+	HIPCHK(c, hipMemcpyAsync(c->dViews.get(), c->hViews, sizeof(DevView) * kMaxViews * n_items, hipMemcpyHostToDevice, s));
+	HIPCHK(c, hipMemcpyAsync(c->dItems.get(), c->hItems, sizeof(EstConst) * n_items, hipMemcpyHostToDevice, s));
+	HIPCHK(c, hipMemcpyAsync(c->dInit.get(), c->hInit, sizeof(InitItem) * n_items, hipMemcpyHostToDevice, s));
+	HIPCHK(c, hipEventRecord(c->tabEv[c->tabSet], s));
 	HIPCHK(c, hipMemsetAsync(c->evals.get(), 0, 64, s));
 	HIPCHK(c, hipMemsetAsync(c->sync.get(), 0, 64 + sizeof(int32_t) * 2 * kMaxBatch, s));
 
 	HIPCHK(c, hipEventRecord(c->ev[0], s));
+	const InitArgs ia{c->dItems.get<EstConst>(), c->dInit.get<InitItem>(), n_items};
 	for (int i = 0; i < n_items; ++i) {
 		const EstConst& k = c->hItems[i];
-		const float* depthIn = items[i].d_depth;
 		if (k.keep) launch_apply_mask(k.keep, items[i].d_depth, items[i].d_normal, k.W * k.H, s);
-		if (p->median_blur) {
-			launch_median3(items[i].d_depth, c->slots[i].tmpDepth.get<float>(), k.W, k.H, s);
-			depthIn = c->slots[i].tmpDepth.get<float>();
-		}
-		launch_score_pass(k, depthIn, items[i].d_normal, c->evals.get<unsigned long long>(), s);
+	}
+	if (p->median_blur) launch_median3(ia, maxW, maxH, s);
+	{
+		const bool two = k_two(items[0].n_src);
+		const int inst = (batch.big ? 4 : 0) | (two ? 2 : 0) | (mask ? 1 : 0);
+		int grid = 4096, nClass = 1;
+		if (c->scoreTileW > 0) {
+			if (c->scoreBlocksPerCU[inst] < 0) c->scoreBlocksPerCU[inst] = score_pass_blocks_per_cu(batch.big, two, mask);
+			nClass = 8;
+			grid = c->scoreBlocksPerCU[inst] > 0 ? c->scoreBlocksPerCU[inst] * c->nCU / 8 * 8 : 4096;
+			if (grid < 8) grid = 8;
+		}
+		launch_score_pass(ia, batch.big, two, mask, nTiles, grid, nClass, c->evals.get<unsigned long long>(), s);
 	}
 	HIPCHK(c, hipEventRecord(c->ev[1], s));
 	int32_t* sync = c->sync.get<int32_t>();
 	const SweepArgs sa{c->dItems.get<EstConst>(), n_items, maxRows, {sync + 16, sync + 16 + kMaxBatch, sync + 1, c->evals.get<unsigned long long>()}, c->sweepLag, c->xcdAffinity};
 	const std::vector<hcmvs::SweepLaunch> plan = hcmvs::plan_sweeps(batch);
 	for (const hcmvs::SweepLaunch& l : plan) {
-		HIPCHK(c, hipMemsetAsync(sync + 16, 0, sizeof(int32_t) * 2 * kMaxBatch, s));
-		for (int i = 0; i < n_items; ++i)
-			HIPCHK(c, hipMemsetAsync(c->slots[i].progress.get(), 0, (size_t)batch.items[i].rows * kProgressStride * sizeof(int32_t), s));
+		launch_clear_progress(ia, sync + 16, 2 * kMaxBatch, s);
 		if (!launch_sweep(sa, l, s))
 			return fail(c, HCMVS_ERR_INVALID, "estimate: no sweep kernel for %d waves per row, big %d two %d pack %d hint %d mask %d spread %d",
 			            l.v.nw, l.v.big, l.v.two, l.v.pack, l.v.hint, l.v.mask, l.v.spread);
 	}
 	c->lastSweepLaunches = (int)plan.size();
 	HIPCHK(c, hipEventRecord(c->ev[2], s));
-	for (int i = 0; i < n_items; ++i)
-		launch_end_pass(c->hItems[i], p->it_external == p->n_external_iters - 1 ? 1 : 0, items[i].d_depth, items[i].d_normal, items[i].d_conf, s);
+	launch_end_pass(ia, p->it_external == p->n_external_iters - 1 ? 1 : 0, s);
 	HIPCHK(c, hipEventRecord(c->ev[3], s));
 	HIPCHK(c, hipGetLastError());
 	c->lastSweeps = p->n_estimation_iters;
diff --git a/hc-mvs_amd/csrc/pm_common.h b/hc-mvs_amd/csrc/pm_common.h
--- a/hc-mvs_amd/csrc/pm_common.h
+++ b/hc-mvs_amd/csrc/pm_common.h
@@ -58,6 +58,18 @@
 	const SpreadView* spread;
 };
 
+struct InitItem {
+	const float* medianIn;
+	float* medianOut;
+	const float* depthIn;
+	const float* normalIn;
+	float *depthOut, *normalOut, *confOut;
+	int32_t tile0;
+	int32_t tilesX;
+	int32_t tw, th;
+	int32_t pad_;
+};
+
 struct SweepSync {
 	int32_t* ticket;
 	int32_t* rowsDone;
@@ -72,16 +84,23 @@
 	int lag, affinity;
 };
 
+struct InitArgs {
+	const EstConst* dItems;
+	const InitItem* dInit;
+	int nItems;
+};
+
 void launch_gray_to_u8(const float* gray, uint8_t* out, int n, hipStream_t s);
 void launch_bgr_to_u8(const uint8_t* bgr, uint8_t* out, int n, hipStream_t s);
 void launch_gradient_map(const uint8_t* g8, uint8_t* gra, int W, int H, hipStream_t s);
-void launch_median3(const float* in, float* out, int W, int H, hipStream_t s);
+void launch_median3(const InitArgs& a, int maxW, int maxH, hipStream_t s);
 void launch_apply_mask(const uint8_t* keep, float* depth, float* normal, int n, hipStream_t s);
 void launch_quads(const float* gray, float4* out, int W, int H, hipStream_t s);
-void launch_score_pass(const EstConst& c, const float* depthIn, const float* normalIn, unsigned long long* evals,
-                       hipStream_t s);
+void launch_score_pass(const InitArgs& a, bool big, bool two, bool mask, int nTiles, int grid, int nClass, unsigned long long* evals, hipStream_t s);
+int score_pass_blocks_per_cu(bool big, bool two, bool mask);
+void launch_clear_progress(const InitArgs& a, int32_t* counters, int nCounters, hipStream_t s);
 bool launch_sweep(const SweepArgs& a, const SweepLaunch& l, hipStream_t s);
-void launch_end_pass(const EstConst& c, int finalPass, float* depth, float* normal, float* conf, hipStream_t s);
+void launch_end_pass(const InitArgs& a, int finalPass, hipStream_t s);
 
 }
 #endif
diff --git a/hc-mvs_amd/csrc/pm_kernels.hip b/hc-mvs_amd/csrc/pm_kernels.hip
--- a/hc-mvs_amd/csrc/pm_kernels.hip
+++ b/hc-mvs_amd/csrc/pm_kernels.hip
@@ -1476,82 +1476,107 @@
 }
 
 
-__global__ void import_kernel(EstConst c, const float* depthIn, const float* normalIn) {
-	const int n = c.W * c.H;
+__global__ void import_kernel(const EstConst* __restrict__ items, const InitItem* __restrict__ init) {
+	const EstConst& c = items[blockIdx.y];
+	gcfptr depthIn = (gcfptr)init[blockIdx.y].depthIn, normalIn = (gcfptr)init[blockIdx.y].normalIn;
+	const HC_GLOBAL uint8_t* keep = as_global(c.keep);
+	HC_GLOBAL f32x4* dn = (HC_GLOBAL f32x4*)c.dn;
+	HC_GLOBAL float* conf = as_global(c.conf);
+	const int W = c.W, H = c.H, border = c.border;
+	const int n = W * H;
 	for (int i = blockIdx.x * blockDim.x + threadIdx.x; i < n; i += gridDim.x * blockDim.x) {
-		const int x = i % c.W, y = i / c.W;
-		const bool inb = x >= c.border && y >= c.border && x < c.W - c.border && y < c.H - c.border;
-		if (c.keep && !c.keep[i]) {
-			c.dn[i] = make_float4(depthIn[i], 0.f, 0.f, 0.f);
-			c.conf[i] = 0.f;
+		const int x = i % W, y = i / W;
+		const bool inb = x >= border && y >= border && x < W - border && y < H - border;
+		if (keep && !keep[i]) {
+			dn[i] = f32x4{depthIn[i], 0.f, 0.f, 0.f};
+			conf[i] = 0.f;
 		} else if (inb) {
-			c.dn[i] = make_float4(depthIn[i], normalIn[3 * i], normalIn[3 * i + 1], normalIn[3 * i + 2]);
-			c.conf[i] = 2.f;
+			dn[i] = f32x4{depthIn[i], normalIn[3 * i], normalIn[3 * i + 1], normalIn[3 * i + 2]};
+			conf[i] = 2.f;
 		} else {
-			c.dn[i] = make_float4(0.f, 0.f, 0.f, 0.f);
-			c.conf[i] = 2.f;
+			dn[i] = f32x4{0.f, 0.f, 0.f, 0.f};
+			conf[i] = 2.f;
 		}
 	}
 }
 
 template <int S, bool BIG, bool TWO = false, bool MASK = false>
-__global__ __launch_bounds__(256) void score_kernel(EstConst c, unsigned long long* evalsOut) {
-	LaneCtx<S> L;
-	lane_init<S>(c, L);
+__global__ __launch_bounds__(256) void score_kernel(const EstConst* __restrict__ items, const InitItem* __restrict__ init, int nItems, int nTiles, int nClass,
+                                                    unsigned long long* evalsOut) {
 	__shared__ float stage[4][3][8][8];
 	__shared__ float bigTab[BIG ? 4 : 1][4][BIG ? kBigSlots : 1];
-	RegStore<S> st;
-	st.stage = stage[threadIdx.x >> 6]; st.seg = L.seg;
-	st.bw = (float (*)[kBigSlots])(BIG ? &bigTab[BIG ? (threadIdx.x >> 6) : 0][0][0] : nullptr);
-	st.put_view(as_global(c.views) + (L.vact ? L.view : 0), L.seg);
-	LaneCtx<S> L1 = L;
-	RegStore<S> st1 = st;
-	if constexpr (TWO) {
-		lane_init<S>(c, L1, 64 / S);
-		st1.put_view(as_global(c.views) + (L1.vact ? L1.view : 0), L1.seg);
-	}
-	const int nrows = c.H - 2 * c.border, ncols = c.W - 2 * c.border;
-	const int total = nrows * ncols;
+	const int wv = threadIdx.x >> 6;
 	const int wavesPerBlock = blockDim.x >> 6;
-	const int gw = blockIdx.x * wavesPerBlock + (threadIdx.x >> 6), nw = gridDim.x * wavesPerBlock;
+	const int cls = (int)blockIdx.x % nClass;
+	const int cw = __builtin_amdgcn_readfirstlane(((int)blockIdx.x / nClass) * wavesPerBlock + wv);
+	const int ncw = ((int)gridDim.x / nClass) * wavesPerBlock;
+	LaneCtx<S> L, L1;
+	RegStore<S> st, st1;
 	unsigned evals = 0;
 	unsigned long long taps = 0;
-	const uint32_t stream0 = (uint32_t)c.itExternal * 64u;
-	for (int p = gw; p < total; p += nw) {
-		const int x = c.border + p % ncols, y = c.border + p / ncols;
-		const int idx = y * c.W + x;
-		if constexpr (MASK) if (!uniform_byte(c.keep, idx)) continue;
-		const uint32_t rk = rand_key(c.seed, (uint32_t)idx, stream0);
-		PixIn<S> in;
-		in.tx = (float)c.gra[idx];
-		load_patch_inputs<S>(c, L, x, y, in);
-		Patch<S> P;
-		fill_patch<S, BIG>(c, L, x, y, in, P, st);
-		PixelGeom G;
-		pixel_geom(c, x, y, G);
-		const float4 cur = c.dn[idx];
-		float d = cur.x, n0 = cur.y, n1 = cur.z, n2 = cur.w;
-		if (!(c.dMin <= d && d < c.dMax)) {
-			d = random_depth(c, rand_unit(rk, 0u));
-			random_normal(G, rand_unit(rk, 1u), rand_unit(rk, 2u), n0, n1, n2);
-		} else if (dot3(n0, n1, n2, G.v0, G.v1, 1.f) >= 0.f) {
-			random_normal(G, rand_unit(rk, 1u), rand_unit(rk, 2u), n0, n1, n2);
-		}
-		float m1 = __builtin_huge_valf(), m2 = __builtin_huge_valf();
-		score_pixel<S, BIG>(c, L, P, st, G.v0, G.v1, 1.f, d, n0, n1, n2, m1, m2);
-		if constexpr (TWO) {
-			st1.copy_patch(st);
-			score_pixel<S, BIG>(c, L1, P, st1, G.v0, G.v1, 1.f, d, n0, n1, n2, m1, m2);
-		}
-		const float s = two_best(c, m1, m2);
-		++evals;
-		taps += (unsigned)((P.a + 1) * (P.a + 1));
-		if (L.lane == 0) {
-			c.dn[idx] = make_float4(d, n0, n1, n2);
-			c.conf[idx] = s;
-		}
-	}
-	if (L.lane == 0 && evals) {
+	int cur = 0, loaded = -1;
+	int first = cw;
+	for (int t = cls; t < nTiles; t += nClass) {
+		while (cur + 1 < nItems && t >= init[cur + 1].tile0) ++cur;
+		const EstConst& c = items[cur];
+		const InitItem& ti = init[cur];
+		const int nrows = c.H - 2 * c.border, ncols = c.W - 2 * c.border;
+		const int lt = t - ti.tile0;
+		const int tx0 = (lt % ti.tilesX) * ti.tw, ty0 = (lt / ti.tilesX) * ti.th;
+		const int tw = ncols - tx0 < ti.tw ? ncols - tx0 : ti.tw, th = nrows - ty0 < ti.th ? nrows - ty0 : ti.th;
+		const int npx = tw * th;
+		int q = first;
+		first = (first + ncw - npx % ncw) % ncw;
+		if (q >= npx) continue;
+		if (loaded != cur) {
+			loaded = cur;
+			lane_init<S>(c, L);
+			st.stage = stage[wv]; st.seg = L.seg;
+			st.bw = (float (*)[kBigSlots])(BIG ? &bigTab[BIG ? wv : 0][0][0] : nullptr);
+			st.put_view(as_global(c.views) + (L.vact ? L.view : 0), L.seg);
+			if constexpr (TWO) {
+				L1 = L; st1 = st;
+				lane_init<S>(c, L1, 64 / S);
+				st1.put_view(as_global(c.views) + (L1.vact ? L1.view : 0), L1.seg);
+			}
+		}
+		const uint32_t stream0 = (uint32_t)c.itExternal * 64u;
+		for (; q < npx; q += ncw) {
+			const int x = c.border + tx0 + q % tw, y = c.border + ty0 + q / tw;
+			const int idx = y * c.W + x;
+			if constexpr (MASK) if (c.keep && !uniform_byte(c.keep, idx)) continue;
+			const uint32_t rk = rand_key(c.seed, (uint32_t)idx, stream0);
+			PixIn<S> in;
+			in.tx = (float)uniform_byte(c.gra, idx);
+			load_patch_inputs<S>(c, L, x, y, in);
+			Patch<S> P;
+			fill_patch<S, BIG>(c, L, x, y, in, P, st);
+			PixelGeom G;
+			pixel_geom(c, x, y, G);
+			const f32x4 cur4 = ((const HC_GLOBAL f32x4*)c.dn)[idx];
+			float d = cur4.x, n0 = cur4.y, n1 = cur4.z, n2 = cur4.w;
+			if (!(c.dMin <= d && d < c.dMax)) {
+				d = random_depth(c, rand_unit(rk, 0u));
+				random_normal(G, rand_unit(rk, 1u), rand_unit(rk, 2u), n0, n1, n2);
+			} else if (dot3(n0, n1, n2, G.v0, G.v1, 1.f) >= 0.f) {
+				random_normal(G, rand_unit(rk, 1u), rand_unit(rk, 2u), n0, n1, n2);
+			}
+			float m1 = __builtin_huge_valf(), m2 = __builtin_huge_valf();
+			score_pixel<S, BIG>(c, L, P, st, G.v0, G.v1, 1.f, d, n0, n1, n2, m1, m2);
+			if constexpr (TWO) {
+				st1.copy_patch(st);
+				score_pixel<S, BIG>(c, L1, P, st1, G.v0, G.v1, 1.f, d, n0, n1, n2, m1, m2);
+			}
+			const float s = two_best(c, m1, m2);
+			++evals;
+			taps += (unsigned)((P.a + 1) * (P.a + 1));
+			if (L.lane == 0) {
+				((HC_GLOBAL f32x4*)c.dn)[idx] = f32x4{d, n0, n1, n2};
+				as_global(c.conf)[idx] = s;
+			}
+		}
+	}
+	if ((threadIdx.x & 63) == 0 && evals) {
 		atomicAdd(evalsOut, (unsigned long long)evals);
 		atomicAdd(evalsOut + 1, (unsigned long long)evals);
 		atomicAdd(evalsOut + 2, taps);
@@ -1588,19 +1613,36 @@
 template __global__ void probe_patch_kernel<8>(EstConst, PixIn<8>, Patch<8>*, RegStore<8>*);
 #endif
 
-__global__ void end_kernel(EstConst c, int finalPass, float* depth, float* normal, float* conf) {
+__global__ void end_kernel(const EstConst* __restrict__ items, const InitItem* __restrict__ init, int finalPass) {
+	const EstConst& c = items[blockIdx.y];
+	HC_GLOBAL float* depth = as_global(init[blockIdx.y].depthOut);
+	HC_GLOBAL float* normal = as_global(init[blockIdx.y].normalOut);
+	HC_GLOBAL float* conf = as_global(init[blockIdx.y].confOut);
+	const HC_GLOBAL uint8_t* keep = as_global(c.keep);
+	const HC_GLOBAL f32x4* dn = (const HC_GLOBAL f32x4*)c.dn;
+	const HC_GLOBAL float* cconf = as_global(c.conf);
+	const float thKeep = c.thKeep;
 	const int n = c.W * c.H;
 	for (int i = blockIdx.x * blockDim.x + threadIdx.x; i < n; i += gridDim.x * blockDim.x) {
-		float4 v = c.dn[i];
-		float cf = c.conf[i];
-		if (finalPass && !(c.keep && !c.keep[i])) {
-			if (v.x <= 0.f || cf >= c.thKeep) { v = make_float4(0.f, 0.f, 0.f, 0.f); cf = 0.f; }
+		f32x4 v = dn[i];
+		float cf = cconf[i];
+		if (finalPass && !(keep && !keep[i])) {
+			if (v.x <= 0.f || cf >= thKeep) { v = f32x4{0.f, 0.f, 0.f, 0.f}; cf = 0.f; }
 			else cf = cf >= 1.f ? 0.f : 1.f - cf;
 		}
 		depth[i] = v.x;
 		normal[3 * i] = v.y; normal[3 * i + 1] = v.z; normal[3 * i + 2] = v.w;
 		conf[i] = cf;
 	}
+}
+
+__global__ void clear_progress_kernel(const EstConst* __restrict__ items, int32_t* counters, int nCounters) {
+	const EstConst& c = items[blockIdx.y];
+	HC_GLOBAL int32_t* w = as_global(c.progress);
+	const int n = (c.H - 2 * c.border) * kProgressStride;
+	for (int i = blockIdx.x * blockDim.x + threadIdx.x; i < n; i += gridDim.x * blockDim.x) w[i] = 0;
+	if (blockIdx.y == 0 && blockIdx.x == 0)
+		for (int i = threadIdx.x; i < nCounters; i += blockDim.x) counters[i] = 0;
 }
 
 
@@ -1641,9 +1683,12 @@
 	const float i00 = g[(size_t)y * W + x], i10 = g[(size_t)y * W + x1], i01 = g[(size_t)y1 * W + x], i11 = g[(size_t)y1 * W + x1];
 	out[(size_t)y * W + x] = make_float4(i00, i10 - i00, i01, i11 - i01);
 }
-__global__ void median3_kernel(const float* in, float* out, int W, int H) {
+__global__ void median3_kernel(const EstConst* __restrict__ items, const InitItem* __restrict__ init) {
+	const int W = items[blockIdx.z].W, H = items[blockIdx.z].H;
 	const int x = blockIdx.x * blockDim.x + threadIdx.x, y = blockIdx.y * blockDim.y + threadIdx.y;
 	if (x >= W || y >= H) return;
+	gcfptr in = (gcfptr)init[blockIdx.z].medianIn;
+	HC_GLOBAL float* out = as_global(init[blockIdx.z].medianOut);
 	float v[9];
 	int n = 0;
 #pragma unroll
@@ -1687,8 +1732,8 @@
 void launch_quads(const float* gray, float4* out, int W, int H, hipStream_t s) {
 	hipLaunchKernelGGL(quad_kernel, dim3((W + 63) / 64, (H + 3) / 4), dim3(64, 4), 0, s, gray, out, W, H);
 }
-void launch_median3(const float* in, float* out, int W, int H, hipStream_t s) {
-	hipLaunchKernelGGL(median3_kernel, dim3((W + 63) / 64, (H + 3) / 4), dim3(64, 4), 0, s, in, out, W, H);
+void launch_median3(const InitArgs& a, int maxW, int maxH, hipStream_t s) {
+	hipLaunchKernelGGL(median3_kernel, dim3((maxW + 63) / 64, (maxH + 3) / 4, a.nItems), dim3(64, 4), 0, s, a.dItems, a.dInit);
 }
 void launch_apply_mask(const uint8_t* keep, float* depth, float* normal, int n, hipStream_t s) {
 	hipLaunchKernelGGL(apply_mask_kernel, dim3(2048), dim3(256), 0, s, keep, depth, normal, n);
@@ -1696,16 +1741,24 @@
 
 template <class K, int N>
 struct KernelTable { K at[N]; };
-using ScoreKernel = void (*)(EstConst, unsigned long long*);
+using ScoreKernel = void (*)(const EstConst*, const InitItem*, int, int, int, unsigned long long*);
 template <int... I>
 static constexpr KernelTable<ScoreKernel, sizeof...(I)> score_table(std::integer_sequence<int, I...>) {
 	return {{score_kernel<8, (I & 4) != 0, (I & 2) != 0, (I & 1) != 0>...}};
 }
 static constexpr auto kScoreKernels = score_table(std::make_integer_sequence<int, 8>{});
-void launch_score_pass(const EstConst& c, const float* depthIn, const float* normalIn, unsigned long long* evals,
-                       hipStream_t s) {
-	hipLaunchKernelGGL(import_kernel, dim3(2048), dim3(256), 0, s, c, depthIn, normalIn);
-	hipLaunchKernelGGL(kScoreKernels.at[(c.adapthalfwin > kHalfWindow ? 4 : 0) | (c.V > 8 ? 2 : 0) | (c.keep ? 1 : 0)], dim3(4096), dim3(256), 0, s, c, evals);
+static dim3 batch_grid(int nItems) { return dim3(nItems >= 8 ? 256 : 2048, nItems); }
+void launch_score_pass(const InitArgs& a, bool big, bool two, bool mask, int nTiles, int grid, int nClass, unsigned long long* evals, hipStream_t s) {
+	hipLaunchKernelGGL(import_kernel, batch_grid(a.nItems), dim3(256), 0, s, a.dItems, a.dInit);
+	hipLaunchKernelGGL(kScoreKernels.at[(big ? 4 : 0) | (two ? 2 : 0) | (mask ? 1 : 0)], dim3(grid), dim3(256), 0, s, a.dItems, a.dInit, a.nItems, nTiles, nClass, evals);
+}
+int score_pass_blocks_per_cu(bool big, bool two, bool mask) {
+	int n = 0;
+	if (hipOccupancyMaxActiveBlocksPerMultiprocessor(&n, kScoreKernels.at[(big ? 4 : 0) | (two ? 2 : 0) | (mask ? 1 : 0)], 256, 0) != hipSuccess) n = 0;
+	return n;
+}
+void launch_clear_progress(const InitArgs& a, int32_t* counters, int nCounters, hipStream_t s) {
+	hipLaunchKernelGGL(clear_progress_kernel, dim3(8, a.nItems), dim3(256), 0, s, a.dItems, counters, nCounters);
 }
 
 using SweepKernel = void (*)(const EstConst*, int, int, SweepSync, int, int, int, int, int);
@@ -1732,8 +1785,8 @@
 	return true;
 }
 
-void launch_end_pass(const EstConst& c, int finalPass, float* depth, float* normal, float* conf, hipStream_t s) {
-	hipLaunchKernelGGL(end_kernel, dim3(2048), dim3(256), 0, s, c, finalPass, depth, normal, conf);
-}
-
-}
+void launch_end_pass(const InitArgs& a, int finalPass, hipStream_t s) {
+	hipLaunchKernelGGL(end_kernel, batch_grid(a.nItems), dim3(256), 0, s, a.dItems, a.dInit, finalPass);
+}
+
+}
```

Result: no change. 22.82 Mpix/s (-0.2%).
